# buggyyang/CDC_compression

Hardware: AMD Instinct MI355X
Metric: decoded images/sec at 256x256, 500-step x-param (higher is better)
Workload: dtype f32 (f16x2 split products)

## Files before the change

### cdc_compression_amd/csrc/cdc_internal.h

```cpp
#pragma once
#include <stdio.h>
#include <string.h>
#include <stdlib.h>
#include <hip/hip_runtime.h>
#include <map>
#include <mutex>
#include <utility>
#include <stdint.h>

#include <string>
#include <vector>

#include "conv_args.h"

extern "C" char **environ;

namespace cdc {

typedef void (*conv_kernel_fn)(const ConvArgs);
conv_kernel_fn conv_lookup_a(int MB, int NPW, int lnmode);
conv_kernel_fn conv_lookup_b(int MB, int NPW, int lnmode);
conv_kernel_fn conv_lookup_c(int MB, int NPW, int lnmode);
conv_kernel_fn conv_lookup_split(int MB, int NPW);
conv_kernel_fn conv_lookup_split2(int MB, int NPW, int lnmode, int xu = 1);
conv_kernel_fn conv_lookup_split2h(int MB, int NPW, int lnmode, int xu = 1);
conv_kernel_fn conv_lookup_split2hu(int MB, int NPW);

struct ConvShape {
    int Cin, Cout, KH, KW, stride;
    int C0 = 0;
    int Win = 0;
    int nz = 1, pad_x[4] = {0, 0, 0, 0};
    bool allow_split = false;
    int arith = 0;
    bool per_image_w = false;
    int Ho, Wo;
    int B;
    bool need_all_cout;
    int lnmode;
    int max_ksplit = 1;
};
bool conv_make_plan(const ConvShape &s, ConvPlan *plan);
hipError_t conv_launch(ConvArgs a, const ConvPlan &plan, int B, int nz, hipStream_t st);

struct PfShape {
    int Cin, Cout, C0 = 0, KH, KW, nz = 1, Ho, Wo, B;
    bool need_all_cout = false;
    int stride = 1;
    int uf = 0;
    int cop = 0;
    int tz = 1;
};
struct PfPlan {
    int MB, NPW, WM, WP, ring, tiles_x, tiles_y, groups; size_t lds_bytes; int lin = 0;
    int x16 = 0;
    int pf3_epv = 0, pf3_G = 0, pf3_iters = 0;
};
bool pf_make_plan(const PfShape &s, PfPlan *plan);
hipError_t pf_launch(PfArgs a, const PfPlan &plan, int B, int nz, hipStream_t st);
bool pf3_make_plan(const PfArgs &a, int B, int nz, PfPlan *plan);
hipError_t pf3_launch(PfArgs a, const PfPlan &plan, int B, hipStream_t st);
int device_cus();
struct WsPlan { int W, NPB, stride, waves, tiles, groups; size_t lds_bytes; };
struct WsArgs;
bool ws_make_plan(int Cin, int C0, int Cout, int H, int W, int B, int stride, WsPlan *plan);
hipError_t ws_launch(WsArgs a, const WsPlan &plan, hipStream_t st);
struct Ws1Plan { int NPB, waves, tiles, groups; size_t lds_bytes; };
struct Ws1Args;
bool ws1_make_plan(int Cin, int C0, int Cout, int HW, int B, bool per_image_w, Ws1Plan *plan);
hipError_t ws1_launch(Ws1Args a, const Ws1Plan &plan, hipStream_t st);
bool pw_make_plan(const PfShape &s, PfPlan *plan);
hipError_t pw_launch(PfArgs a, const PfPlan &plan, int B, hipStream_t st);
hipError_t pf_pack_launch(const float *src, long long src_bs, void *dst, long long dst_bs, int C, int H, int W, int B,
                          hipStream_t st);
hipError_t c4_pack_launch(const float *src, long long src_bs, float *dst, int C, long long HW, int B, hipStream_t st);
hipError_t pf_unpack_launch(const void *src, long long src_bs, float *dst, long long dst_bs, int C, int H, int W, int B, hipStream_t st);

inline const char *dev_env(const char *name) {
    static const bool on = [] {
        const char *e = ::getenv("CDC_DEV");
        if (e && atoi(e) != 0) return true;
        static const char *const user_level[] = {"CDC_DEV=", "CDC_ARITH=", "CDC_NO_RANGE_GUARD=", "CDC_GRAPH=", "CDC_DEBUG_PLAN=", "CDC_PROF_OPS=",
                                                 "CDC_BENCH_", "CDC_TEST_OBS=", "CDC_SYNC_EACH_OP=", "CDC_HIP_LIB=", "CDC_NO_COMBINE_FUSE="};
        for (char **v = environ; v && *v; ++v) {
            if (strncmp(*v, "CDC_", 4)) continue;
            bool user = false;
            for (const char *u : user_level) user = user || !strncmp(*v, u, strlen(u));
            if (!user) {
                fprintf(stderr, "cdc_hip: %.*s is set but ignored: development switches need CDC_DEV=1\n", (int)strcspn(*v, "="), *v);
                break;
            }
        }
        return false;
    }();
    return on ? ::getenv(name) : nullptr;
}

inline hipError_t ensure_dynamic_lds(const void *fn, size_t bytes) {
    if (bytes <= 64 * 1024) return hipSuccess;
    static std::mutex mu;
    static std::map<std::pair<int, const void *>, size_t> done;
    int dev = 0;
    (void)hipGetDevice(&dev);
    std::lock_guard<std::mutex> lk(mu);
    size_t &have = done[{dev, fn}];
    if (have >= bytes) return hipSuccess;
    hipError_t e = hipFuncSetAttribute(fn, hipFuncAttributeMaxDynamicSharedMemorySize, (int)bytes);
    if (e == hipSuccess) have = bytes;
    return e;
}

__host__ __device__ inline int ceil_div(int a, int b) { return (a + b - 1) / b; }
__host__ __device__ inline int round_up(int a, int b) { return ceil_div(a, b) * b; }

struct LnArgs {
    const float *in;
    float *out;
    int C, HW;
    const float *g, *b;
    float eps;
    int relu;
    const float *shift;
    int shift_bs;
    const float *resid;
    float *stat_mean, *stat_rstd;
    int nparts;
    long long part_stride;
    int *fault;
    int img_major;
};
hipError_t ln_launch(const LnArgs &a, int B, hipStream_t st);

struct TembLayer {
    const float *w, *bias;
    int cout;
    int out_off;
};
struct TembArgs {
    const float *time;
    const float *w0, *b0;
    const float *w2, *b2;
    int dim;
    const TembLayer *layers;
    int n_layers;
    float *shift;
    int shift_bs;
};
hipError_t temb_launch(const TembArgs &a, int B, hipStream_t st);

struct KvCtxArgs {
    const float *x; long long x_bs;
    const float *mean, *rstd;
    const float *Wt;
    const float *bias;
    const unsigned short *Ws;
    int C, N, nsplit;
    float *S, *Z, *M;
    int f16 = 0;
    float wscale_inv = 1.f;
};
hipError_t kvctx_launch(const KvCtxArgs &a, int B, hipStream_t st);

struct LnConvArgs {
    const float *x; long long x_bs;
    const float *mean, *rstd;
    const unsigned short *Ws;
    const float *bias;
    float *y; long long y_bs;
    int C, N, nsplit;
    void *y_pf = nullptr;
    long long pf_bs = 0, pf_ps = 0;
    int W = 0;
};
hipError_t lnconv_launch(const LnConvArgs &a, int B, hipStream_t st);

hipError_t kstats_launch(const float *k, long long k_bs, int C, int N, float *kmax, int B,
                         hipStream_t st);
hipError_t ctx_partial_launch(const float *k, const float *v, long long kv_bs, int C, int N,
                              const float *kmax, float *S, float *Zp, int nsplit, int B,
                              hipStream_t st, int f16 = 0);
hipError_t ctx_one_launch(const float *k, const float *v, long long kv_bs, int C, int N, float scale, float *ctxw, int Cin_pad, int COP,
                          unsigned short *Ws, int B, hipStream_t st, int f16);
hipError_t ctx_reduce_launch(const float *S, const float *ksum, int C, int nsplit, float scale,
                             float *ctxw, int Cin_pad, int COP, int B, hipStream_t st, unsigned short *Ws = nullptr);

hipError_t ctx_fold_launch(const float *S, const float *ksum, int C, int nsplit, float scale,
                           const float *WoT, const float *WqT, float *T1, float *Mt, int Cin_pad,
                           int COP, const float *ln_g, const float *u, const float *b_out,
                           float *biasB, int B, hipStream_t st, const float *M = nullptr,
                           unsigned short *Ws = nullptr, int ws_f16 = 0, const float *Wq = nullptr);
hipError_t fold_combine_launch(const float *P, const float *bias, float *out, int Cout, int KH,
                               int pad, int H, int W, int B, hipStream_t st);

struct DdimArgs {
    const float *fx, *x, *noise;
    float *x_next;
    const float *tab;
    int steps, i;
    const int *step_ptr;
    int pred_mode, clip;
    float eta;
    long long n;
    long long clip_half_n;
    int *fault;
    const float *tab_v;
    const float *P = nullptr, *P_bias = nullptr;
    int pC = 0, pKH = 0, pPad = 0, pH = 0, pW = 0;
    const unsigned long long *seeds = nullptr;
    long long per_image = 0;
};
hipError_t ddim_launch(const DdimArgs &a, hipStream_t st);
hipError_t randn_fill_launch(const unsigned long long *seeds, int B, long long per_image, unsigned draw, float scale, float *out,
                             hipStream_t st);
hipError_t copy_channels_launch(const float *src, long long src_bs, float *dst, long long dst_bs,
                                long long n, int B, hipStream_t st, int parts = 1, long long part_stride = 0,
                                const int *step_ptr = nullptr, long long step_stride = 0);
hipError_t step_dec_launch(int *step, hipStream_t st);
hipError_t bpp_launch(const float *qh, long long nh, int hw_h, const float *prior, const float *ql, const float *mean,
                      const float *scale, long long nl, float inv_hw, float *bpp, int B, hipStream_t st);
hipError_t clamp_min_launch(float *x, long long bs, long long n, float lo, int B, hipStream_t st);
hipError_t nonfinite_launch(const float *x, long long bs, long long n, int B, int *flag, hipStream_t st);
hipError_t bits_differ_launch(const float *a, const float *b, long long n, long long *counters, hipStream_t st);
hipError_t dequantize_launch(const float *x, const float *loc, float *out, long long n, hipStream_t st);
hipError_t vbr_affine_launch(float *x, long long bs, int C, int HW, const float *rate, const float *p, int leaky, int B, hipStream_t st);
hipError_t frame_in_launch(const void *src, int u8, float *dst, int P, int H, int W, int Hp, int Wp, int zero, hipStream_t st);
hipError_t frame_out_launch(const float *src, void *dst, int u8, int P, int H, int W, int Hp, int Wp, hipStream_t st);
hipError_t unfold_x_launch(const float *src, long long src_bs, float *dst, long long dst_bs, int C, int KW,
                           int pad, int H, int W, int B, hipStream_t st);

}
```

### cdc_compression_amd/csrc/cdc_planner.hip

```cpp
#include "cdc_state.h"

namespace cdcapi {

constexpr int kKsTarget = 1024;

struct Builder {
    cdc_handle *h;
    int B;
    std::vector<void *> *pool;
    int rc = CDC_OK;
    int planB = 0;
    int pb() const { return planB > 0 ? planB : B; }
    std::vector<Op> *cur = nullptr;

    int ws1_h = 0;
    void emit(Op op) {
        op.id = (int)h->op_ms.size();
        h->op_ms.push_back(0); h->op_n.push_back(0); h->op_flops.push_back(op.flops);
        char buf[160];
        const char *kinds[] = {"conv", "ln", "temb", "kstats", "ctxp", "ctxr", "ctxf", "combine", "ddim", "copy", "unfold", "kvctx", "lnconv", "convpf", "pfpack", "convws", "convws1", "vbr"};
        if (op.kind == Op::PFPACK && op.pk.c4 == 2) kinds[Op::PFPACK] = "pfunpack";
        if (op.kind == Op::CONV)
            snprintf(buf, sizeof buf, "conv %dx%d s%d %4d->%-4d out %3dx%-3d MB%d NPW%d WN%d g%d tg%d ipw%d ks%d%s%s%s%s%s", op.conv.KH,
                     op.conv.KW, op.conv.stride, op.conv.Cin, op.conv.Cout, op.conv.Ho, op.conv.Wo, op.plan.MB,
                     op.plan.NPW, op.plan.WN, op.plan.groups, op.plan.tg, op.plan.ipw, op.plan.ksplit, op.plan.split == 2 ? (op.plan.arith ? " SPLIT2H" : " SPLIT2") : (op.plan.split ? " SPLIT" : ""),
                     op.conv.ep_g ? " LN" : "",
                     op.conv.ln_mean ? " pre" : "", cur == &h->pre_ops ? " HOIST" : "", op.conv.resid ? " +res" : "");
        else if (op.kind == Op::CONVPF)
            snprintf(buf, sizeof buf, "conv %dx%d s%d %4d->%-4d out %3dx%-3d MB%d NPW%d WM%d WP%d g%d R%d %s%s%s%s%s%s", op.pf.KH, op.pf.KW,
                     op.pf.stride == 2 ? 2 : 1, op.pf.Cin, op.pf.Cout, op.pf.Ho, op.pf.Wo, op.pfplan.MB, op.pfplan.NPW, op.pfplan.WM, op.pfplan.WP,
                     op.pfplan.groups, op.pfplan.ring, op.pw ? (op.pf.pre_mean ? "PW pre" : "PW") : (op.pfplan.pf3_epv ? (op.pf.ep_g ? "PF3 LN" : "PF3") : (op.pf.ep_g ? "PF LN" : "PF")), op.pf.out ? "" : " nof32", op.pf.out_pf ? " +pf" : "",
                     op.pf.resid ? " +res" : (op.pf.resid_pf ? " +resP" : ""), cur == &h->pre_ops ? " HOIST" : "", op.pf.tz == 4 ? " TZ4" : "");
        else if (op.kind == Op::CONVWS)
            snprintf(buf, sizeof buf, "conv 3x3 s%d %4d->%-4d out %3dx%-3d NPB%d waves%d tiles%d g%d WS%s", op.wsplan.stride, op.ws.Cin, op.ws.Cout, op.ws.H, op.wsplan.W,
                     op.wsplan.NPB, op.wsplan.waves, op.wsplan.tiles, op.wsplan.groups, op.ws.pre_add ? " pre_add" : "");
        else if (op.kind == Op::CONVWS1)
            snprintf(buf, sizeof buf, "conv 1x1 s1 %4d->%-4d out %3dx%-3d NPB%d waves%d tiles%d g%d WS1%s%s%s", op.ws1.Cin, op.ws1.Cout, ws1_h, op.ws1.HW / std::max(ws1_h, 1),
                     op.ws1plan.NPB, op.ws1plan.waves, op.ws1plan.tiles, op.ws1plan.groups, op.ws1.pre_mean ? " pre" : "", op.ws1.w_bs ? " perimg" : "",
                     op.ws1.resid ? (op.ws1.resid_is_pre ? " pre_add" : " +res") : "");
        else if (op.kind == Op::LN)
            snprintf(buf, sizeof buf, "ln C=%d HW=%d%s", op.ln.C, op.ln.HW, op.ln.out ? "" : " stats");
        else if (op.kind == Op::KVCTX)
            snprintf(buf, sizeof buf, "kvctx C=%d N=%d nsplit=%d", op.kvc.C, op.kvc.N, op.kvc.nsplit);
        else if (op.kind == Op::LNCONV)
            snprintf(buf, sizeof buf, "lnconv C=%d N=%d nsplit=%d", op.lnc.C, op.lnc.N, op.lnc.nsplit);
        else if (op.kind == Op::VBR)
            snprintf(buf, sizeof buf, "vbr C=%d HW=%d%s", op.vb.C, op.vb.HW, op.vb.leaky ? " leaky" : "");
        else if (op.kind == Op::KSTATS || op.kind == Op::CTXP || op.kind == Op::CTXR || op.kind == Op::CTXF)
            snprintf(buf, sizeof buf, "%s C=%d N=%d nsplit=%d", op.at_one ? "ctx1" : kinds[op.kind], op.at.C, op.at.N, op.at_one ? 1 : op.at.nsplit);
        else
            snprintf(buf, sizeof buf, "%s", kinds[op.kind]);
        if (cur == &h->pre_ops && !strstr(buf, " HOIST") && strlen(buf) + 7 < sizeof buf) strcat(buf, " HOIST");
        h->op_label.push_back(buf);
        (cur ? cur : &h->ops)->push_back(op);
    }

    int *fault_flag() {
        if (!h->d_fault && !rc) {
            void *p = nullptr;
            hipError_t e = hipMalloc(&p, sizeof(int));
            if (e == hipSuccess) e = hipMemset(p, 0, sizeof(int));
            if (e != hipSuccess) { rc = fail(h, CDC_ERR_NOMEM, "range-guard flag: %s", hipGetErrorString(e)); return nullptr; }
            h->d_fault = (int *)p;
            h->weight_allocs.push_back(p);
        }
        return h->d_fault;
    }

    float *dalloc(size_t nfloats) {
        if (rc) return nullptr;
        void *p = nullptr;
        const size_t bytes = std::max<size_t>(nfloats, 1) * sizeof(float);
        hipError_t e = hipMalloc(&p, bytes);
        if (e != hipSuccess) {
            rc = fail(h, CDC_ERR_NOMEM, "hipMalloc(%zu bytes) failed: %s", bytes, hipGetErrorString(e));
            return nullptr;
        }
        pool->push_back(p);
        h->act_bytes += bytes;
        return (float *)p;
    }
    struct PfTwin { void *p = nullptr; int C = 0, H = 0, W = 0; bool valid = false;
                    bool only = false;
                    long long ps() const { return (long long)(H + 2) * (W + 2); }
                    long long bs() const { return (long long)(C / 8) * 2 * ps(); } };
    std::map<const float *, PfTwin> pfmap;
    enum Site { SITE_NONE, SITE_ALWAYS, SITE_RB_CHAIN, SITE_DOWN, SITE_JOIN, SITE_ALWAYS_PLANES };
    int pf_mode() const { const char *e = dev_env("CDC_PF"); return h->arith != 1 ? 0 : (e ? atoi(e) : 3); }
    bool pf_site(Site s, int H, int W) const {
        const int m = pf_mode();
        if (m == 1) return s != SITE_NONE;
        if (m != 3) return false;
        const long long join_max = 16384;
        return s == SITE_RB_CHAIN || s == SITE_DOWN || s == SITE_ALWAYS_PLANES || (s == SITE_JOIN && (long long)H * W <= join_max);
    }
    bool pf_on() const { return pf_mode() != 0; }
    static long long pf_maxpix() { const char *e = dev_env("CDC_PF_MAXPIX"); const long long v = e ? atoll(e) : 0; return v > 0 ? v : (1LL << 40); }
    PfTwin *twin(const float *p) { auto it = pfmap.find(p); return it == pfmap.end() ? nullptr : &it->second; }
    bool still_planes_only(const float *p) { PfTwin *t = twin(p); return t && t->only; }
    void add_twin(const float *p, int C, int H, int W) {
        if (rc || !p || !pf_on() || (C % 16) || W < 32 || H < 2 || (long long)H * W > pf_maxpix()) return;
        PfTwin t; t.C = C; t.H = H; t.W = W;
        const size_t bytes = (size_t)B * t.bs() * 16;
        void *q = nullptr;
        hipError_t e = hipMalloc(&q, bytes);
        if (e == hipSuccess) e = hipMemset(q, 0, bytes);
        if (e != hipSuccess) { rc = fail(h, CDC_ERR_NOMEM, "PF tensor (%zu bytes): %s", bytes, hipGetErrorString(e)); return; }
        pool->push_back(q);
        h->act_bytes += bytes;
        t.p = q;
        pfmap[p] = t;
    }
    void pack(const float *p, long long bs) {
        PfTwin *t = twin(p);
        if (rc || !t) return;
        Op op; op.kind = Op::PFPACK; op.prof = PC_SMALL;
        op.pk = {p, bs, t->p, t->bs(), t->C, t->H, t->W, 0};
        op.bytes = 8.0 * B * t->C * t->H * t->W;
        emit(op);
        t->valid = true;
    }
    bool ensure_f32(const float *q, long long bs) {
        PfTwin *t = q ? twin(q) : nullptr;
        if (!t || !t->only) return true;
        if (rc || !t->valid || bs != (long long)t->C * t->H * t->W) return false;
        Op op; op.kind = Op::PFPACK; op.prof = PC_SMALL;
        op.pk = {q, bs, t->p, t->bs(), t->C, t->H, t->W, 2};
        op.bytes = 8.0 * B * t->C * t->H * t->W;
        emit(op);
        t->only = false;
        ++n_unpacked;
        if (debug_plan()) fprintf(stderr, "[plan] planes-only tensor %dx%dx%d unpacked for an fp32 reader\n", t->C, t->H, t->W);
        return true;
    }
    int n_unpacked = 0;

    std::map<const float *, float *> c4map;
    const float *pre_add_c4(const float *p, int C, int H, int W, long long bs) {
        if (rc || (C % 4) || bs != (long long)C * H * W || dev_env("CDC_NO_PRE_C4")) return nullptr;
        auto it = c4map.find(p);
        if (it != c4map.end()) return it->second;
        float *q = dalloc((size_t)B * C * H * W);
        if (rc) return nullptr;
        std::vector<Op> *saved = cur;
        cur = &h->pre_ops;
        Op op; op.kind = Op::PFPACK; op.prof = PC_SMALL;
        op.pk = {p, bs, q, 0, C, H, W, 1};
        op.bytes = 8.0 * B * C * H * W;
        emit(op);
        cur = saved;
        c4map[p] = q;
        return q;
    }
    Act new_act(int C, int H, int W, bool want_twin = true, Site site = SITE_ALWAYS) {
        Act a; a.C = C; a.H = H; a.W = W;
        a.p = dalloc((size_t)B * C * H * W);
        if (want_twin && pf_site(site, H, W)) add_twin(a.p, C, H, W);
        return a;
    }

    struct ConvOpts {
        const float *ln_g = nullptr, *ln_b = nullptr;
        int relu = 0;
        float relu_slope = 0.f;
        const float *shift = nullptr;
        const float *resid = nullptr; long long resid_bs = 0, resid_cs = 0;
        const float *resid1 = nullptr; long long resid1_bs = 0; int resid_c0 = 0;
        const float *pre_add = nullptr;
        float *stat_mean = nullptr, *stat_rstd = nullptr;
        const float *pre_mean = nullptr, *pre_rstd = nullptr, *pre_g = nullptr, *pre_b = nullptr;
        int pre_mode = 1;
        int shift_bs = -1;
        long long w_bs = 0;
        long long wsp_bs = 0;
        bool no_bias = false;
        const float *res3_w = nullptr, *res3_x = nullptr; long long res3_bs = 0;
        int max_ksplit = 1;
        bool emit_pf = false;
        bool pf_only = false;
        bool no_f32 = false;
        int uf_c = 0, uf_pad = 0;
        bool linear_epilogue() const { return !ln_g && !relu && !shift && !stat_mean && !pre_add && !res3_w; }
    };
    int last_ksplit = 1;
    bool last_pf_only = false;
    const float *next_res3_w = nullptr, *next_res3_x = nullptr; long long next_res3_bs = 0;
    static bool debug_plan() { return getenv("CDC_DEBUG_PLAN") != nullptr; }

    PfShape pf_shape(const ConvW &w, int C0, int Ho, int Wo, bool need_all) const {
        PfShape ps;
        ps.Cin = w.Cin; ps.Cout = w.Cout; ps.C0 = C0; ps.KH = w.KH; ps.KW = w.KW; ps.nz = w.nz; ps.Ho = Ho; ps.Wo = Wo; ps.B = pb();
        ps.need_all_cout = need_all; ps.cop = w.COP;
        return ps;
    }
    bool pf_form(const ConvW &w, int C0, int H, int W, bool need_all, PfShape *ps) const {
        if (!w.wsh || w.stride != 1 || w.transposed || (w.Cin % 16) || !((w.KH == 3 && w.KW == 3) || (w.KH == 1 && w.KW == 1))) return false;
        if (w.py() != w.KH / 2 || w.px() != w.KW / 2) return false;
        *ps = pf_shape(w, C0, H, W, need_all);
        return true;
    }
    bool pf_s2_form(const ConvW &w, int C0, int H, int W, bool need_all, PfShape *ps) const {
        if (!w.wsh || w.stride != 2 || w.transposed || w.KH != 3 || w.KW != 3 || C0 || (H & 1) || (W & 1) || (w.Cin % 16)) return false;
        if (w.py() != 1 || w.px() != 1) return false;
        *ps = pf_shape(w, 0, H / 2, W / 2, need_all);
        ps->stride = 2;
        return true;
    }
    bool pf_tz_form(const ConvW &w, int C0, int H, int W, bool need_all, PfShape *ps) const {
        if (!w.wsh || !w.transposed || w.tk != 4 || w.KH != 2 || w.KW != 2 || C0 || (w.Cin % 16)) return false;
        *ps = pf_shape(w, 0, H, W, need_all);
        ps->tz = 4;
        return true;
    }
    bool pf_17_form(const ConvW &w, int C0, int H, int W, bool need_all, PfShape *ps) const {
        if (!w.wsh || w.KH != 1 || w.KW != 7 || w.stride != 1 || w.transposed || C0 || (w.Cin % 16)) return false;
        if (w.py() != 0 || w.px() != 3) return false;
        *ps = pf_shape(w, 0, H, W, need_all);
        return true;
    }
    bool pf_uf_form(const ConvW &w, int H, int W, bool need_all, PfShape *ps) const {
        if (!w.wsh || w.KH != 7 || w.KW != 1 || w.stride != 1 || w.transposed || w.nz != 1 || w.py() != 3 || w.px() != 0) return false;
        *ps = pf_shape(w, 0, H, W, need_all);
        ps->uf = 3;
        return true;
    }
    bool pw_form(const ConvW &w, int C0, int H, int W, PfShape *ps) const {
        if (!w.wsh || w.KH != 1 || w.KW != 1 || w.stride != 1 || w.transposed || w.nz != 1 || w.py() != 0 || w.px() != 0) return false;
        *ps = pf_shape(w, C0, H, W, false);
        return true;
    }
    static bool pf_plans(const PfShape &ps) { PfPlan plan; return pf_make_plan(ps, &plan); }

    bool pf_would_plan(const ConvW &w, int H, int W) { PfShape ps; return pf_on() && pf_form(w, 0, H, W, true, &ps) && pf_plans(ps); }
    bool pf_s2_would_plan(const ConvW &w, int H, int W) { PfShape ps; return pf_on() && pf_s2_form(w, 0, H, W, false, &ps) && pf_plans(ps); }
    bool pf_tz_would_plan(const ConvW &w, int H, int W) { PfShape ps; return pf_on() && pf_tz_form(w, 0, H, W, false, &ps) && pf_plans(ps); }
    bool pf_17_would_plan(const ConvW &w, int H, int W) { PfShape ps; return pf_on() && pf_17_form(w, 0, H, W, false, &ps) && pf_plans(ps); }

    bool join_reads_planes(const ResBlockW &rb, const float *p0, int C0, const float *p1, int H, int W) {
        PfTwin *t0 = twin(p0), *t1 = twin(p1);
        if (!t0 || !t1 || !t1->valid || t0->H != H || t0->W != W || t1->H != H || t1->W != W) return false;
        if (t0->C != C0 || t0->C + t1->C != rb.c1.Cin) return false;
        return join_would_read_planes(rb, C0, H, W);
    }
    bool join_would_read_planes(const ResBlockW &rb, int C0, int H, int W) {
        if (!pf_on() || !rb.has_res || rb.hoist_cx) return false;
        if (rb.cres.Cin != rb.c1.Cin || (C0 % 16) || C0 <= 0 || C0 >= rb.c1.Cin || !pf_site(SITE_JOIN, H, W)) return false;
        PfShape p1, pr;
        return pf_form(rb.c1, C0, H, W, rb.c1.KH == 3, &p1) && pf_plans(p1) && pf_form(rb.cres, C0, H, W, rb.cres.KH == 3, &pr) && pf_plans(pr);
    }

    template <class A> static void out_geometry(A &a, const ConvW &w, int Ho, int Wo) {
        if (w.transposed) {
            for (int z = 0; z < 4; ++z) {
                const int py = z >> 1, px = z & 1;
                a.pad_y[z] = w.tk == 5 ? 1 : 1 - py; a.pad_x[z] = w.tk == 5 ? 1 : 1 - px;
                a.out_zoff[z] = py * 2 * Wo + px;
            }
            a.out_cs = (long long)4 * Ho * Wo; a.out_ys = 4 * Wo; a.out_xs = 2;
        } else {
            a.pad_y[0] = w.py(); a.pad_x[0] = w.px();
            a.out_cs = (long long)Ho * Wo; a.out_ys = Wo; a.out_xs = 1;
        }
        a.Ho = Ho; a.Wo = Wo;
    }
    PfTwin *out_twin(const float *out, long long bs, int C, int H, int W) {
        PfTwin *t = twin(out);
        return t && t->C == C && t->H == H && t->W == W && bs == (long long)C * H * W ? t : nullptr;
    }
    template <class A> bool bind_out_pf(A &a, const ConvW &w, const float *out, long long out_bs, int Ho, int Wo) {
        const int Wt = w.transposed ? 2 * Wo : Wo;
        PfTwin *to = out_twin(out, out_bs, w.Cout, w.transposed ? 2 * Ho : Ho, Wt);
        if (!to) return false;
        a.out_pf = to->p; a.pf_bs = to->bs(); a.pf_ps = to->ps();
        if (w.transposed) {
            a.pf_ys = 2 * (Wt + 2); a.pf_xs = 2;
            for (int z = 0; z < 4; ++z) a.pf_zoff[z] = ((z >> 1) + 1) * (Wt + 2) + (z & 1) + 1;
        } else {
            a.pf_ys = Wt + 2; a.pf_xs = 1; a.pf_zoff[0] = (Wt + 2) + 1;
        }
        to->valid = true;
        return true;
    }
    int shift_stride(const ConvOpts &o) const { return o.shift_bs >= 0 ? o.shift_bs : h->shift_bs; }
    template <class A> void epilogue(A &a, const ConvW &w, const ConvOpts &o) {
        a.bias = o.no_bias ? nullptr : w.bias;
        a.pre_add = o.pre_add;
        a.ep_g = o.ln_g; a.ep_b = o.ln_b; a.eps = 1e-5f; a.relu = o.relu; a.relu_slope = o.relu_slope;
        a.shift = o.shift; a.shift_bs = shift_stride(o);
        a.resid = o.resid; a.resid_bs = o.resid_bs; a.resid_cs = o.resid_cs;
        a.stat_mean = o.stat_mean; a.stat_rstd = o.stat_rstd;
        a.res3_w = o.res3_w; a.res3_x = o.res3_x; a.res3_bs = o.res3_bs;
        a.fault = fault_flag();
    }
    bool finish(Op &op, double flops, double bytes, bool pf_only) {
        op.flops = flops; op.bytes = bytes;
        last_ksplit = 1;
        last_pf_only = pf_only;
        emit(op);
        return true;
    }

    bool try_pf(const ConvW &w, const float *s0, int C0, const float *s1, int H, int W, float *out, long long out_bs,
                const ConvOpts &o, bool need_all, int prof) {
        if (!pf_on() || o.pre_mean || o.w_bs || o.wsp_bs || o.max_ksplit > 1) return false;
        PfShape ps;
        const int c0 = s1 ? C0 : 0;
        if (!(pf_form(w, c0, H, W, need_all, &ps) || (pf_s2_form(w, c0, H, W, need_all, &ps) && !o.pre_add && !o.res3_w) ||
              pf_tz_form(w, c0, H, W, need_all, &ps) || (pf_17_form(w, c0, H, W, need_all, &ps) && !o.ln_g && !o.emit_pf)))
            return false;
        if (s1 && dev_env("CDC_TEST_JOIN_MISS")) return false;
        PfTwin *t0 = twin(s0), *t1 = s1 ? twin(s1) : nullptr;
        if (!t0 || !t0->valid || (s1 && (!t1 || !t1->valid))) return false;
        if (t0->H != H || t0->W != W || (t1 && (t1->H != H || t1->W != W))) return false;
        if (s1 ? (t0->C != C0 || t0->C + t1->C != w.Cin) : t0->C != w.Cin) return false;
        PfPlan plan;
        if (!pf_make_plan(ps, &plan)) return false;
        const int Ho = ps.Ho, Wo = ps.Wo;
        Op op;
        op.kind = Op::CONVPF; op.prof = prof; op.pfplan = plan; op.nz = w.nz;
        PfArgs &a = op.pf;
        memset(&a, 0, sizeof a);
        a.src0 = t0->p; a.src0_bs = t0->bs();
        if (t1) { a.src1 = t1->p; a.src1_bs = t1->bs(); }
        a.C0 = s1 ? C0 : w.Cin; a.Cin = w.Cin; a.H = H; a.W = W;
        a.w = w.wsh; a.w_zs = w.wsp_zs / 8;
        a.KH = w.KH; a.KW = w.KW; a.nz = w.nz; a.stride = w.stride; a.tz = ps.tz;
        a.nchunk = w.Cin / 16; a.COP = w.COP; a.Cout = w.Cout;
        a.acc_scale = w.wscale_inv;
        out_geometry(a, w, Ho, Wo);
        a.out = out; a.out_bs = out_bs;
        if (o.emit_pf && bind_out_pf(a, w, out, out_bs, Ho, Wo) && o.no_f32) a.out = nullptr;
        epilogue(a, w, o);
        if (o.resid1) {
            if (!o.resid || o.resid_c0 <= 0 || o.resid_c0 >= w.Cout || (o.resid_c0 % 64) || (o.resid_c0 % (plan.MB * 32))) return false;
            a.resid1 = o.resid1; a.resid1_bs = o.resid1_bs; a.resid_c0 = o.resid_c0;
        }
        if (PfTwin *tr = o.resid ? twin(o.resid) : nullptr)
            if (tr->only) {
                if (!tr->valid || tr->C != w.Cout || tr->H != Ho || tr->W != Wo || w.transposed || w.stride != 1 ||
                    o.resid_bs != (long long)w.Cout * Ho * Wo || o.resid_cs != (long long)Ho * Wo) {
                    if (!ensure_f32(o.resid, o.resid_bs)) {
                        if (!rc) rc = fail(h, CDC_ERR_UNSUPPORTED, "planes-only residual of a shape the plane-operand kernels do not read");
                        return true;
                    }
                } else {
                    a.resid = nullptr;
                    a.resid_pf = tr->p; a.rpf_bs = tr->bs(); a.rpf_ps = tr->ps(); a.rpf_ys = Wo + 2; a.rpf_zoff = (Wo + 2) + 1;
                }
            }
        if (planB == 0) pf3_make_plan(a, B, w.nz, &op.pfplan);
        if (debug_plan())
            fprintf(stderr, "[plan] conv %dx%d %d->%d out %dx%d on conv_pf%s_kernel (epv %d, %d workgroups x %d tiles per group)\n", w.KH, w.KW, w.Cin, w.Cout,
                    Ho, Wo, op.pfplan.pf3_epv ? "3" : "", op.pfplan.pf3_epv, op.pfplan.pf3_G, op.pfplan.pf3_iters);
        const double px = (double)B * Ho * Wo * w.nz;
        return finish(op, 2.0 * px * w.Cout * w.Cin * w.KH * w.KW, 4.0 * ((double)B * w.Cin * H * W + px * w.Cout), a.out == nullptr);
    }

    bool try_pf_uf(const ConvW &w, const float *s0, long long bs0, int H, int W, float *out, long long out_bs, const ConvOpts &o,
                   bool need_all, int prof) {
        PfShape ps;
        if (!pf_on() || o.uf_c != 3 || o.uf_pad != 3 || !pf_uf_form(w, H, W, need_all, &ps)) return false;
        if (o.pre_mean || o.w_bs || o.wsp_bs || o.max_ksplit > 1 || o.resid || o.res3_w || o.stat_mean) return false;
        PfPlan plan;
        if (!pf_make_plan(ps, &plan)) return false;
        Op op;
        op.kind = Op::CONVPF; op.prof = prof; op.pfplan = plan; op.nz = 1;
        PfArgs &a = op.pf;
        memset(&a, 0, sizeof a);
        a.x0 = s0; a.x0_bs = bs0;
        a.C0 = a.Cin = 32; a.H = H; a.W = W;
        a.w = w.wsh; a.w_zs = w.wsp_zs / 8;
        a.KH = 7; a.KW = 1; a.nz = 1;
        a.nchunk = 2; a.COP = w.COP; a.Cout = w.Cout;
        a.acc_scale = w.wscale_inv;
        out_geometry(a, w, H, W);
        a.out = out; a.out_bs = out_bs;
        if (o.emit_pf && bind_out_pf(a, w, out, out_bs, H, W) && o.no_f32) a.out = nullptr;
        const float *c4 = o.pre_add && cur != &h->pre_ops ? pre_add_c4(o.pre_add, w.Cout, H, W, out_bs) : nullptr;
        epilogue(a, w, o);
        if (c4) { a.pre_add = c4; a.pre_c4 = 1; }
        const double px = (double)B * H * W;
        return finish(op, 2.0 * px * w.Cout * w.Cin * 7, 4.0 * ((double)B * 3 * H * W + px * w.Cout), a.out == nullptr);
    }

    bool try_pw(const ConvW &w, const float *s0, int C0, long long bs0, const float *s1, long long bs1, int H, int W,
                float *out, long long out_bs, const ConvOpts &o, bool need_all, int prof) {
        PfShape ps;
        if (h->arith != 1 || dev_env("CDC_NO_PW") || !pw_form(w, s1 ? C0 : 0, H, W, &ps)) return false;
        if (need_all || o.ln_g || o.stat_mean || o.res3_w || o.pf_only) return false;
        if (o.pre_mean && o.pre_mode != 2) return false;
        if (o.w_bs && !o.wsp_bs) return false;
        PfPlan plan;
        if (!pw_make_plan(ps, &plan)) return false;
        if (plan.lin && (o.shift || o.wsp_bs || (long long)w.Cout * H * W != out_bs)) return false;
        if (debug_plan())
            fprintf(stderr, "[plan] conv1x1 PW Cin=%4d Cout=%4d out=%3dx%-3d %s%s| MB=%d NPW=%d WM=%d WP=%d groups=%d R=%d wgs=%d lds=%zu\n", w.Cin, w.Cout,
                    H, W, o.pre_mean ? "pre2 " : "", o.wsp_bs ? "per-image " : "", plan.MB, plan.NPW, plan.WM, plan.WP, plan.groups, plan.ring,
                    plan.tiles_x * plan.tiles_y * B * plan.groups, plan.lds_bytes);
        Op op;
        op.kind = Op::CONVPF; op.prof = prof; op.pfplan = plan; op.nz = 1; op.pw = true;
        PfArgs &a = op.pf;
        memset(&a, 0, sizeof a);
        a.x0 = s0; a.x0_bs = bs0; a.x1 = s1; a.x1_bs = bs1;
        a.C0 = s1 ? C0 : w.Cin; a.Cin = w.Cin; a.H = H; a.W = W;
        a.pre_mean = o.pre_mean; a.pre_rstd = o.pre_mean ? o.pre_rstd : nullptr;
        a.w = w.wsh; a.w_bs = o.wsp_bs / 8;
        a.KH = 1; a.KW = 1; a.nz = 1;
        a.nchunk = w.Cin / 16; a.COP = w.COP; a.Cout = w.Cout;
        a.acc_scale = w.wscale_inv;
        out_geometry(a, w, H, W);
        a.out = out; a.out_bs = out_bs;
        if (o.emit_pf && !plan.lin && (w.Cout % 32) == 0 && bind_out_pf(a, w, out, out_bs, H, W) && o.no_f32) a.out = nullptr;
        epilogue(a, w, o);
        const double px = (double)B * H * W;
        return finish(op, 2.0 * px * w.Cout * w.Cin, 4.0 * ((double)B * w.Cin * H * W + px * w.Cout), a.out == nullptr);
    }

    bool ws_would_plan(const ConvW &w, int C0, bool two_src, int H, int W, WsPlan *plan) {
        if (h->arith != 1 || !w.wsh || planB > 0 || w.KH != 3 || w.KW != 3 || (w.stride != 1 && w.stride != 2) || w.transposed || w.nz != 1) return false;
        if (w.py() != 1 || w.px() != 1) return false;
        if (w.COP != w.Cout || w.Cin_pad != w.Cin) return false;
        if (w.stride == 2 && ((H & 1) || (W & 1) || two_src)) return false;
        return ws_make_plan(w.Cin, two_src ? C0 : w.Cin, w.Cout, H / w.stride, W / w.stride, pb(), w.stride, plan);
    }
    bool try_ws(const ConvW &w, const float *s0, int C0, long long bs0, const float *s1, long long bs1, int H, int W, float *raw,
                long long raw_bs, int prof, const float *pre_add = nullptr) {
        Op op;
        op.kind = Op::CONVWS; op.prof = prof;
        if (rc || !ws_would_plan(w, C0, s1 != nullptr, H, W, &op.wsplan)) return false;
        if (!ensure_f32(s0, bs0) || (s1 && !ensure_f32(s1, bs1))) return false;
        const int Ho = H / w.stride, Wo = W / w.stride;
        if (raw_bs != (long long)w.Cout * Ho * Wo) return false;
        WsArgs &a = op.ws;
        memset(&a, 0, sizeof a);
        a.x0 = s0; a.x0_bs = bs0; a.x1 = s1; a.x1_bs = bs1;
        a.C0 = s1 ? C0 : w.Cin; a.Cin = w.Cin; a.H = Ho; a.B = B;
        a.w = w.wsh; a.nchunk = w.Cin / 16; a.COP = w.COP; a.Cout = w.Cout; a.acc_scale = w.wscale_inv;
        a.bias = pre_add ? nullptr : w.bias;
        a.pre_add = pre_add;
        a.out = raw; a.out_bs = raw_bs;
        a.fault = fault_flag();
        if (debug_plan())
            fprintf(stderr, "[plan] conv 3x3 s%d %d->%d out %dx%d on conv_ws_kernel: %d tiles of %d pixels x %d groups, %d waves, %zu bytes of LDS\n", w.stride, w.Cin, w.Cout, Ho, Wo,
                    op.wsplan.tiles, op.wsplan.NPB * 32, op.wsplan.groups, op.wsplan.waves, op.wsplan.lds_bytes);
        const double px = (double)B * Ho * Wo;
        return finish(op, 2.0 * px * w.Cout * w.Cin * 9, 4.0 * ((double)B * H * W * w.Cin + px * w.Cout), false);
    }

    bool try_ws1(const ConvW &w, const float *s0, int C0, long long bs0, const float *s1, long long bs1, int H, int W, float *out, long long out_bs,
                 const ConvOpts &o, bool need_all, int prof) {
        PfShape ps;
        if (rc || h->arith != 1 || planB > 0 || !pw_form(w, 0, H, W, &ps)) return false;
        if (need_all || o.ln_g || o.stat_mean || o.res3_w || o.pf_only || (o.pre_add && o.resid) || o.relu || o.resid1 || o.uf_c) return false;
        if (o.pre_mean && o.pre_mode != 2) return false;
        if (o.w_bs && !o.wsp_bs) return false;
        if (w.COP != w.Cout || w.Cin_pad != w.Cin || out_bs != (long long)w.Cout * H * W) return false;
        if (o.resid && (o.resid_cs != (long long)H * W)) return false;
        const long long blocks = (long long)pb() * (H * W / 32);
        const long long max_blocks = dev_env("CDC_WS1_MAX_BLOCKS") ? atoll(dev_env("CDC_WS1_MAX_BLOCKS")) : 128;
        const int max_groups_wide = dev_env("CDC_WS1_MAX_GROUPS") ? atoi(dev_env("CDC_WS1_MAX_GROUPS")) : 0;
        const bool wide_ok = blocks <= max_blocks || (max_groups_wide > 0 && blocks <= 256 && w.Cout / 32 <= max_groups_wide);
        if (!wide_ok && !(o.wsp_bs && W < 32)) return false;
        Op op;
        op.kind = Op::CONVWS1; op.prof = prof;
        if (!ws1_make_plan(w.Cin, s1 ? C0 : w.Cin, w.Cout, H * W, pb(), o.wsp_bs != 0, &op.ws1plan)) return false;
        if (!ensure_f32(s0, bs0) || (s1 && !ensure_f32(s1, bs1)) || (o.resid && !ensure_f32(o.resid, o.resid_bs))) return false;
        Ws1Args &a = op.ws1;
        memset(&a, 0, sizeof a);
        a.x0 = s0; a.x0_bs = bs0; a.x1 = s1; a.x1_bs = bs1;
        a.C0 = s1 ? C0 : w.Cin; a.Cin = w.Cin; a.HW = H * W; a.B = B;
        a.pre_mean = o.pre_mean; a.pre_rstd = o.pre_mean ? o.pre_rstd : nullptr;
        a.w = w.wsh; a.w_bs = o.wsp_bs / 8;
        a.nchunk = w.Cin / 16; a.COP = w.COP; a.Cout = w.Cout; a.acc_scale = w.wscale_inv;
        a.bias = o.no_bias ? nullptr : w.bias;
        a.shift = o.shift; a.shift_bs = shift_stride(o);
        a.resid = o.resid; a.resid_bs = o.resid_bs;
        if (o.pre_add) { a.resid = o.pre_add; a.resid_bs = out_bs; a.resid_is_pre = 1; }
        a.out = out; a.out_bs = out_bs;
        a.fault = fault_flag();
        if (debug_plan())
            fprintf(stderr, "[plan] conv 1x1 %d->%d out %dx%d on conv_ws1_kernel: %d tiles of %d pixels x %d groups, %d waves%s%s\n", w.Cin, w.Cout, H, W,
                    op.ws1plan.tiles, op.ws1plan.NPB * 32, op.ws1plan.groups, op.ws1plan.waves, o.pre_mean ? ", folded PreNorm" : "", o.wsp_bs ? ", per-image weights" : "");
        ws1_h = H;
        const double px = (double)B * H * W;
        return finish(op, 2.0 * px * w.Cout * w.Cin, 4.0 * px * (w.Cin + w.Cout), false);
    }

    bool conv(const ConvW &w, const float *s0, int C0, long long bs0, const float *s1,
              long long bs1, int H, int W, float *out, long long out_bs, const ConvOpts &o,
              bool need_all, int prof) {
        if (rc) return true;
        if (s1 && (C0 % 4)) {
            const long long n0 = (long long)C0 * H * W, n1 = (long long)(w.Cin - C0) * H * W;
            float *cat = dalloc((size_t)B * (n0 + n1));
            copy(s0, bs0, cat, n0 + n1, n0);
            copy(s1, bs1, cat + n0, n0 + n1, n1);
            s0 = cat; bs0 = n0 + n1; s1 = nullptr; bs1 = 0;
        }
        ConvShape s;
        s.Cin = w.Cin; s.Cout = w.Cout; s.KH = w.KH; s.KW = w.KW; s.stride = w.stride;
        s.C0 = s1 ? C0 : 0;
        s.Win = W; s.nz = w.nz;
        s.allow_split = w.wsp != nullptr;
        s.arith = (h->arith == 1 && w.wsh) ? 1 : 0;
        s.per_image_w = o.wsp_bs != 0;
        for (int z = 0; z < 4; ++z) s.pad_x[z] = w.transposed ? (w.tk == 5 ? 1 : 1 - (z & 1)) : w.px();
        if (w.transposed) { s.Ho = H; s.Wo = W; }
        else {
            s.Ho = (H + 2 * w.py() - w.KH) / w.stride + 1;
            s.Wo = (W + 2 * w.px() - w.KW) / w.stride + 1;
        }
        s.B = pb(); s.need_all_cout = need_all; s.lnmode = o.pre_mean ? o.pre_mode : 0;
        if (!o.uf_c && try_pf(w, s0, C0, s1, H, W, out, out_bs, o, need_all, prof)) return true;
        if (o.uf_c && !s1 && try_pf_uf(w, s0, bs0, H, W, out, out_bs, o, need_all, prof)) return true;
        if (o.pf_only) return false;
        if (o.resid1 && !rc) { rc = fail(h, CDC_ERR_UNSUPPORTED, "a two-source residual reached a kernel without it"); return true; }
        {
            const std::pair<const float *, long long> rd[3] = {{s0, bs0}, {s1, bs1}, {o.resid, o.resid_bs}};
            for (const auto &q : rd)
                if (!ensure_f32(q.first, q.second) && !rc) {
                    rc = fail(h, CDC_ERR_UNSUPPORTED, "a planes-only tensor reached a kernel that reads fp32 and cannot be unpacked");
                    return true;
                }
        }
        if (w.stride == 2 && !need_all && o.linear_epilogue() && !o.resid && !o.pre_mean && !o.w_bs && !o.uf_c && !(o.emit_pf && twin(out)) &&
            try_ws(w, s0, C0, bs0, s1, bs1, H, W, out, out_bs, prof))
            return true;
        if (!o.uf_c && try_ws1(w, s0, C0, bs0, s1, bs1, H, W, out, out_bs, o, need_all, prof)) return true;
        if (!o.uf_c && try_pw(w, s0, C0, bs0, s1, bs1, H, W, out, out_bs, o, need_all, prof)) return true;
        const bool linear_ep = !need_all && o.linear_epilogue() && w.nz == 1 && !w.transposed;
        s.max_ksplit = o.max_ksplit > 1 ? o.max_ksplit : (linear_ep ? 4 : 1);
        if (need_all && (w.Cout % 32)) return false;
        ConvPlan plan;
        if (!conv_make_plan(s, &plan)) {
            if (need_all) return false;
            rc = fail(h, CDC_ERR_UNSUPPORTED, "no launch plan for conv Cin=%d Cout=%d k=%dx%d out=%dx%d",
                      w.Cin, w.Cout, w.KH, w.KW, s.Ho, s.Wo);
            return true;
        }
        if (o.uf_c && !(plan.split == 2 && plan.arith == 1 && plan.xu == 1 && plan.lnmode == 0 &&
                        conv_lookup_split2hu(plan.MB, plan.NPW))) return false;
        last_ksplit = 1;
        last_pf_only = false;
        if (o.max_ksplit > 1 && plan.split == 2 && !need_all) {
            const long long wgs = (long long)(plan.ipw > 1 ? ceil_div(pb(), plan.ipw) : plan.tiles_x * plan.tiles_y * pb()) *
                                  plan.groups * w.nz;
            int ks = (int)std::min<long long>(ceil_div(kKsTarget, wgs), std::min(o.max_ksplit, plan.nchunk / 4));
            if (ks > 1) { plan.ksplit = ks; last_ksplit = ks; }
        }
        float *ks_scratch = nullptr;
        const long long dense_bs = (long long)w.Cout * s.Ho * s.Wo;
        if (o.max_ksplit <= 1 && plan.split == 2 && linear_ep) {
            const long long wgs = (long long)(plan.ipw > 1 ? ceil_div(pb(), plan.ipw) : plan.tiles_x * plan.tiles_y * pb()) *
                                  plan.groups;
            const int ks = (int)std::min<long long>(ceil_div(kKsTarget, wgs), std::min(4, plan.nchunk / 4));
            if (ks > 1 && (planB > 0 || (size_t)B * dense_bs * 4 * ks <= (64u << 20))) {
                plan.ksplit = ks;
                ks_scratch = dalloc((size_t)ks * B * dense_bs);
            }
        }
        if (debug_plan())
            fprintf(stderr, "[plan] %-10s Cin=%4d Cout=%4d k=%dx%d s=%d in=%3dx%-3d out=%3dx%-3d %s%s%s| MB=%2d NPW=%d "
                    "WN=%d groups=%2d KC=%2d nchunk=%3d tiles=%dx%d wgs=%6d lds=%6zu\n", kProfNames[prof], w.Cin,
                    w.Cout, w.KH, w.KW, w.stride, H, W, s.Ho, s.Wo, need_all ? "LN " : "   ",
                    s.lnmode ? (s.lnmode == 2 ? "pre2 " : "pre1 ") : "     ", cur == &h->pre_ops ? "HOIST " : "", plan.MB, plan.NPW, plan.WN,
                    plan.groups, plan.KC, plan.nchunk, plan.tiles_x, plan.tiles_y,
                    plan.tiles_x * plan.tiles_y * B * plan.groups * w.nz, plan.lds_bytes);
        Op op;
        op.kind = Op::CONV; op.prof = prof; op.plan = plan; op.nz = w.nz;
        ConvArgs &a = op.conv;
        memset(&a, 0, sizeof a);
        a.src0 = s0; a.src1 = s1; a.src0_bs = bs0; a.src1_bs = bs1;
        a.C0 = s1 ? C0 : w.Cin; a.Cin = w.Cin; a.H = H; a.W = W;
        a.ln_mean = o.pre_mean; a.ln_rstd = o.pre_rstd; a.ln_g = o.pre_g; a.ln_b = o.pre_b;
        a.wp = w.wp; a.w_bs = o.w_bs; a.w_zs = w.w_zs;
        a.wsp = w.wsp; a.wsp_zs = w.wsp_zs; a.wsp_bs = o.wsp_bs;
        a.acc_scale = 1.f;
        if (plan.split == 2 && plan.arith == 1) { a.wsp = w.wsh; a.acc_scale = w.wscale_inv; }
        a.KH = w.KH; a.KW = w.KW; a.stride = w.stride;
        a.Cin_pad = w.Cin_pad; a.COP = w.COP; a.Cout = w.Cout;
        a.out = out; a.out_bs = out_bs; a.out_ks = (long long)B * out_bs;
        out_geometry(a, w, s.Ho, s.Wo);
        epilogue(a, w, o);
        if (o.uf_c) {
            a.uf_c = o.uf_c; a.uf_pad = o.uf_pad;
            a.uf_magic = o.uf_c > 1 ? (unsigned)(((1ull << 32) + o.uf_c - 1) / o.uf_c) : 0u;
        }
        if (o.emit_pf && !ks_scratch && plan.ksplit <= 1 && (w.Cout % 32) == 0 && bind_out_pf(a, w, out, out_bs, s.Ho, s.Wo)) {
            a.pf_only = o.no_f32 ? 1 : 0;
            last_pf_only = o.no_f32;
        }
        const double px = (double)B * s.Ho * s.Wo * w.nz;
        op.flops = 2.0 * px * w.Cout * w.Cin * w.KH * w.KW;
        op.bytes = 4.0 * ((double)B * w.Cin * H * W + px * w.Cout);
        if (ks_scratch) {
            a.out = ks_scratch; a.out_bs = dense_bs; a.out_ks = (long long)B * dense_bs;
        }
        emit(op);
        if (ks_scratch) {
            Op c; c.kind = Op::COPY; c.prof = prof;
            c.cp = {ks_scratch, dense_bs, out, out_bs, dense_bs};
            c.cp_parts = plan.ksplit; c.cp_part_stride = (long long)B * dense_bs;
            c.bytes = 4.0 * B * dense_bs * (plan.ksplit + 1);
            emit(c);
            if (o.emit_pf && !w.transposed && out_twin(out, out_bs, w.Cout, s.Ho, s.Wo)) pack(out, out_bs);
        }
        return true;
    }

    void ln(const float *in, float *out, int C, int HW, const float *g, const float *b, int relu,
            const float *shift, const float *resid, float *sm, float *sr, int nparts = 1) {
        if (rc) return;
        Op op;
        op.kind = Op::LN; op.prof = PC_LN;
        LnArgs &a = op.ln;
        a.nparts = nparts; a.part_stride = (long long)B * C * HW;
        a.in = in; a.out = out; a.C = C; a.HW = HW; a.g = g; a.b = b; a.eps = 1e-5f; a.relu = relu;
        a.shift = shift; a.shift_bs = h->shift_bs; a.resid = resid; a.stat_mean = sm; a.stat_rstd = sr;
        a.fault = fault_flag();
        op.bytes = 4.0 * B * C * HW * (out ? 2 : 1);
        emit(op);
    }

    void copy(const float *src, long long src_bs, float *dst, long long dst_bs, long long n) {
        Op c; c.kind = Op::COPY; c.prof = PC_SMALL;
        c.cp = {src, src_bs, dst, dst_bs, n};
        c.bytes = 8.0 * B * n;
        emit(c);
    }

    bool prefer_fused(const ConvW &w, int H, int W) {
        if (w.Cout % 32 || w.Cout > 384) return false;
        if (w.wsp && w.Cout > 256 && (W & 3) == 0 && !dev_env("CDC_NO_SPLIT")) return false;
        ConvShape s;
        s.Cin = w.Cin; s.Cout = w.Cout; s.KH = w.KH; s.KW = w.KW; s.stride = w.stride;
        s.Ho = H; s.Wo = W; s.B = pb(); s.lnmode = 0;
        s.Win = W; s.pad_x[0] = w.pad;
        ConvPlan pf, pu;
        s.need_all_cout = true;
        if (!conv_make_plan(s, &pf)) return false;
        s.need_all_cout = false;
        if (!conv_make_plan(s, &pu)) return true;
        const double wf = (double)pf.tiles_x * pf.tiles_y * B * pf.WN;
        const double wu = (double)pu.tiles_x * pu.tiles_y * B * pu.groups * pu.WN;
        static const double thr = 512;
        if (wf >= thr) return true;
        return wu < 1.5 * wf;
    }

    bool block(const ConvW &w, const float *s0, int C0, long long bs0, const float *s1, long long bs1,
               int H, int W, Act out, const float *g, const float *b, const float *shift,
               const float *pre_add, const float *resid, long long resid_bs, float *sm, float *sr,
// ... 769 lines not shown
```

### cdc_compression_amd/csrc/conv_inst_p.hip

```cpp
#include <algorithm>
#include <map>
#include <string>
#include <vector>
#include <stdlib.h>

#include "cdc_internal.h"
#include "conv_pf_kernel.h"

namespace cdc {

template <int KH, int KW>
static pf_kernel_fn pf_lookup_k(int MB, int NPW, int WM, int WP) {
    if (MB == 2 && NPW == 2 && WM == 1 && WP == 4) return conv_pf_kernel<2, 2, 1, 4, KH, KW>;
    if (MB == 2 && NPW == 2 && WM == 2 && WP == 2) return conv_pf_kernel<2, 2, 2, 2, KH, KW>;
    if (MB == 2 && NPW == 2 && WM == 2 && WP == 4) return conv_pf_kernel<2, 2, 2, 4, KH, KW>;
    if (MB == 3 && NPW == 2 && WM == 2 && WP == 4) return conv_pf_kernel<3, 2, 2, 4, KH, KW>;
    if (MB == 3 && NPW == 1 && WM == 2 && WP == 4 && KH == 3) return conv_pf_kernel<3, 1, 2, 4, KH, KW>;
    if (MB == 2 && NPW == 2 && WM == 4 && WP == 2) return conv_pf_kernel<2, 2, 4, 2, KH, KW>;
    return nullptr;
}
static pf_kernel_fn pf_lookup_s2(int MB, int NPW, int WM, int WP) {
    if (MB == 2 && NPW == 1 && WM == 1 && WP == 4) return conv_pf_kernel<2, 1, 1, 4, 3, 3, 2>;
    if (MB == 2 && NPW == 2 && WM == 2 && WP == 2) return conv_pf_kernel<2, 2, 2, 2, 3, 3, 2>;
    if (MB == 3 && NPW == 1 && WM == 2 && WP == 4) return conv_pf_kernel<3, 1, 2, 4, 3, 3, 2>;
    return nullptr;
}
static pf_kernel_fn pf_lookup_tz(int MB, int NPW, int WM, int WP) {
    if (MB == 1 && NPW == 2 && WM == 2 && WP == 2) return conv_pf_kernel<1, 2, 2, 2, 2, 2, 1, 4>;
    if (MB == 2 && NPW == 1 && WM == 1 && WP == 4) return conv_pf_kernel<2, 1, 1, 4, 2, 2, 1, 4>;
    if (MB == 1 && NPW == 2 && WM == 4 && WP == 2) return conv_pf_kernel<1, 2, 4, 2, 2, 2, 1, 4>;
    return nullptr;
}
static pf_kernel_fn pf_lookup(int MB, int NPW, int WM, int WP, int KH, int KW, int stride = 1, int tz = 1) {
    if (tz == 4) return (KH == 2 && KW == 2 && stride != 2) ? pf_lookup_tz(MB, NPW, WM, WP) : nullptr;
    if (stride == 2) return (KH == 3 && KW == 3) ? pf_lookup_s2(MB, NPW, WM, WP) : nullptr;
    if (KH == 3 && KW == 3) return pf_lookup_k<3, 3>(MB, NPW, WM, WP);
    if (KH == 1 && KW == 1) return pf_lookup_k<1, 1>(MB, NPW, WM, WP);
    if (KH == 2 && KW == 2) return pf_lookup_k<2, 2>(MB, NPW, WM, WP);
    if (KH == 1 && KW == 7 && MB == 1 && NPW == 2 && WM == 1 && WP == 4) return conv_pf_kernel<1, 2, 1, 4, 1, 7>;
    if (KH == 7 && KW == 1 && MB == 2 && NPW == 2 && WM == 1 && WP == 4) return conv_pf_kernel<2, 2, 1, 4, 7, 1, 1, 1, 3>;
    return nullptr;
}

struct PfCand { int MB, NPW, WM, WP; };
static const PfCand kCandsS2[] = {
    {2, 2, 2, 2},
    {3, 1, 2, 4},
    {2, 1, 1, 4},
};
static const PfCand kCandsTZ[] = {
    {1, 2, 4, 2},
    {2, 1, 1, 4},
    {1, 2, 2, 2},
};
static const PfCand kCands[] = {
    {2, 2, 4, 2},
    {3, 2, 2, 4},
    {3, 1, 2, 4},
    {2, 2, 2, 2},
    {2, 2, 2, 4},
    {2, 2, 1, 4},
};

bool pf_make_plan(const PfShape &s, PfPlan *p) {
    if (s.uf) {
        if (s.uf != 3 || s.KH != 7 || s.KW != 1 || s.Cin != 21 || s.Cout != 64 || s.cop != 64 || s.C0 || s.nz != 1 || s.stride != 1 || s.tz != 1 ||
            s.Wo < 32 || dev_env("CDC_NO_PF_UF"))
            return false;
        const int ring = pf_ring(2, 2, 1, 4, 7, 1);
        const double wgs = (double)((s.Wo + 31) / 32) * ((s.Ho + 7) / 8) * s.B;
        const double min_wgs = dev_env("CDC_PF_UF_MIN_WGS") ? atof(dev_env("CDC_PF_UF_MIN_WGS")) : 512.0;
        if (ring < 3 || wgs < min_wgs) return false;
        p->MB = 2; p->NPW = 2; p->WM = 1; p->WP = 4; p->ring = ring;
        p->tiles_x = (s.Wo + 31) / 32; p->tiles_y = (s.Ho + 7) / 8; p->groups = 1;
        p->lds_bytes = (size_t)2 * pf_patch_units(2, 4, 7, 1) * 16 + (size_t)ring * pf_rows(2, 2) * 64 * 16 + (size_t)pf_uf_stage_floats(2, 4) * 4;
        return true;
    }
    if (s.KH == 1 && s.KW == 7) {
        if (s.Cout > 32 || s.cop != 32 || s.Cin % 16 || s.C0 || s.nz != 1 || s.stride != 1 || s.tz != 1 || s.need_all_cout || s.Wo < 32 ||
            dev_env("CDC_NO_PF_17"))
            return false;
        const int ring = pf_ring(1, 2, 1, 4, 1, 7);
        const double wgs = (double)((s.Wo + 31) / 32) * ((s.Ho + 7) / 8) * s.B;
        const double min_wgs = dev_env("CDC_PF_17_MIN_WGS") ? atof(dev_env("CDC_PF_17_MIN_WGS")) : 768.0;
        if (!ring || (s.Cin / 16) * 7 < ring - 1 || wgs < min_wgs) return false;
        p->MB = 1; p->NPW = 2; p->WM = 1; p->WP = 4; p->ring = ring;
        p->tiles_x = (s.Wo + 31) / 32; p->tiles_y = (s.Ho + 7) / 8; p->groups = 1;
        p->lds_bytes = (size_t)2 * pf_patch_units(2, 4, 1, 7) * 16 + (size_t)ring * pf_rows(1, 2) * 32 * 16;
        return true;
    }
    if (s.Cout % 32 || s.Cin % 16 || (s.C0 % 16)) return false;
    if (s.Wo < 32) return false;
    const char *force = dev_env("CDC_PF_PLAN");
    int f[4] = {0, 0, 0, 0};
    if (force) sscanf(force, "%d,%d,%d,%d", &f[0], &f[1], &f[2], &f[3]);
    double best = -1;
    if (s.stride == 2) {
        if (s.KH != 3 || s.KW != 3 || s.nz != 1 || s.C0 || dev_env("CDC_NO_PF_S2")) return false;
        for (const PfCand &c : kCandsS2) {
            if (f[0] && (c.MB != f[0] || c.NPW != f[1] || c.WM != f[2] || c.WP != f[3])) continue;
            const int COPT = c.WM * c.MB * 32, TH = c.WP * c.NPW;
            if (s.Cout % COPT || (s.need_all_cout && COPT != s.Cout)) continue;
            const int ring = pf_ring(c.MB, c.NPW, c.WM, c.WP, 3, 3, 2);
            const int tps = pf_tps(c.MB, c.NPW, c.WM, c.WP, 3, 3, 2);
            const int S = (s.Cin / 16) * 9 / tps;
            if (!ring || S < ring - 1) continue;
            const double wgs = (double)((s.Wo + 31) / 32) * ((s.Ho + TH - 1) / TH) * s.B * (s.Cout / COPT);
            const double min_wgs = dev_env("CDC_PF_S2_MIN_WGS") ? atof(dev_env("CDC_PF_S2_MIN_WGS")) : 128.0;
            if (wgs < min_wgs) continue;
            const double score = (double)COPT;
            if (score <= best) continue;
            best = score;
            const size_t patch = (size_t)pf_patch_bufs(3, 3, 2) * pf_patch_units(c.NPW, c.WP, 3, 3, 2) * 16, wst = (size_t)tps * pf_rows(c.MB, c.NPW) * COPT * 16;
            p->MB = c.MB; p->NPW = c.NPW; p->WM = c.WM; p->WP = c.WP;
            p->ring = ring;
            p->tiles_x = (s.Wo + 31) / 32; p->tiles_y = (s.Ho + TH - 1) / TH;
            p->groups = s.Cout / COPT;
            p->lds_bytes = std::max(patch + ring * wst, sizeof(float) * (size_t)(4 * COPT + 2 * c.WM * c.WP * c.NPW * 32));
        }
        return best >= 0;
    }
    if (s.tz == 4) {
        if (s.KH != 2 || s.KW != 2 || s.C0 || dev_env("CDC_NO_PF_TZ")) return false;
        for (const PfCand &c : kCandsTZ) {
            if (f[0] && (c.MB != f[0] || c.NPW != f[1] || c.WM != f[2] || c.WP != f[3])) continue;
            const int COPT = c.WM * c.MB * 32, TH = c.WP * c.NPW;
            if (COPT != s.Cout) continue;
            const int ring = pf_ring(c.MB, c.NPW, c.WM, c.WP, 2, 2, 1, 4);
            const int tps = pf_tps(c.MB, c.NPW, c.WM, c.WP, 2, 2, 1, 4);
            const int S = (s.Cin / 16) * 16 / tps;
            if (!ring || S < ring - 1) continue;
            const double wgs = (double)((s.Wo + 31) / 32) * ((s.Ho + TH - 1) / TH) * s.B;
            const double min_wgs = dev_env("CDC_PF_TZ_MIN_WGS") ? atof(dev_env("CDC_PF_TZ_MIN_WGS")) : 128.0;
            if (wgs < min_wgs) continue;
            best = COPT;
            const size_t patch = (size_t)2 * pf_patch_units(c.NPW, c.WP, 2, 2, 1, 4) * 16, wst = (size_t)tps * pf_rows(c.MB, 4 * c.NPW) * COPT * 16;
            p->MB = c.MB; p->NPW = c.NPW; p->WM = c.WM; p->WP = c.WP;
            p->ring = ring;
            p->tiles_x = (s.Wo + 31) / 32; p->tiles_y = (s.Ho + TH - 1) / TH;
            p->groups = 1;
            p->lds_bytes = std::max(patch + ring * wst, sizeof(float) * (size_t)(4 * COPT + 2 * c.WM * c.WP * 4 * c.NPW * 32));
            break;
        }
        return best >= 0;
    }
    for (const PfCand &c : kCands) {
        if (f[0] && (c.MB != f[0] || c.NPW != f[1] || c.WM != f[2] || c.WP != f[3])) continue;
        const int COPT = c.WM * c.MB * 32, NW = c.WM * c.WP;
        if (s.Cout % COPT) continue;
        if (s.need_all_cout && COPT != s.Cout) continue;
        if (!pf_lookup(c.MB, c.NPW, c.WM, c.WP, s.KH, s.KW)) continue;
        const int TH = c.WP * c.NPW, PH = TH + s.KH - 1, PW = 32 + s.KW - 1;
        const int xsw = (4 * PH * PW + 63) / 64;
        if (xsw > 2 * kPfXS) continue;
        const int taps = s.KH * s.KW, npb = taps == 1 ? 3 : 2;
        const size_t patch = (size_t)npb * xsw * 64 * 16, wst = (size_t)pf_rows(c.MB, c.NPW) * COPT * 16;
        const int ring = pf_ring(c.MB, c.NPW, c.WM, c.WP, s.KH, s.KW);
        if (!ring) continue;
        const int S = (s.Cin / 16) * taps;
        if (S < ring - 1) continue;
        const double wgs = (double)((s.Wo + 31) / 32) * ((s.Ho + TH - 1) / TH) * s.B * (s.Cout / COPT) * s.nz;
        const double min_waves = dev_env("CDC_PF_MIN_WAVES") ? atof(dev_env("CDC_PF_MIN_WAVES")) : 256.0;
        if (wgs * NW < min_waves) continue;
        if (c.MB == 3 && c.NPW == 1 && wgs < 128.0) continue;
        const double fill = std::min(1.0, wgs * NW / 2048.0);
        const double reads = (3.0 * c.MB + 2.0 * c.NPW) / (3.0 * c.MB * c.NPW);
        const double score = fill * (1.0 - 0.35 * reads) * (s.Cout / COPT > 1 ? 0.9 : 1.0);
        if (score > best) {
            best = score;
            p->MB = c.MB; p->NPW = c.NPW; p->WM = c.WM; p->WP = c.WP;
            p->ring = ring;
            p->tiles_x = (s.Wo + 31) / 32; p->tiles_y = (s.Ho + TH - 1) / TH;
            p->groups = s.Cout / COPT;
            p->lds_bytes = std::max(patch + ring * wst, sizeof(float) * (size_t)(4 * COPT + 2 * c.WM * c.WP * c.NPW * 32));
        }
    }
    return best >= 0;
}

hipError_t pf_launch(PfArgs a, const PfPlan &p, int B, int nz, hipStream_t st) {
    if (p.pf3_epv) return pf3_launch(a, p, B, st);
    pf_kernel_fn fn = pf_lookup(p.MB, p.NPW, p.WM, p.WP, a.KH, a.KW, a.stride == 2 ? 2 : 1, a.tz == 4 ? 4 : 1);
    if (!fn) return hipErrorInvalidValue;
    if (a.tz == 4) nz = 1;
    a.lognbw = 5;
    a.dbg = 0;
    a.tiles_x = p.tiles_x; a.tiles_y = p.tiles_y; a.B = B; a.ring = p.ring;
    if (hipError_t e = ensure_dynamic_lds((const void *)fn, p.lds_bytes); e != hipSuccess) return e;
    dim3 grid((unsigned)(p.tiles_x * p.tiles_y * B), (unsigned)p.groups, (unsigned)nz);
    a.xcd_remap = (grid.x % 8 == 0 && grid.x >= 64) ? 1 : 0;
#ifdef CDC_TIMELINE
    static unsigned long long *tl_dev = nullptr;
    static std::map<std::string, int> seen;
    const size_t tl_wgs = (size_t)grid.x * grid.y * grid.z;
    char key[96];
    snprintf(key, sizeof key, "%dx%d s%d tz%d %d->%d out %dx%d", a.KH, a.KW, a.stride == 2 ? 2 : 1, a.tz == 4 ? 4 : 1, a.Cin, a.Cout, a.Ho, a.Wo);
    a.tl = nullptr;
    if (tl_wgs <= (1u << 18) && seen[key]++ < 3) {
        if (!tl_dev) hipMalloc(&tl_dev, sizeof(unsigned long long) * 16 * (1u << 18));
        hipMemsetAsync(tl_dev, 0, sizeof(unsigned long long) * 16 * tl_wgs, st);
        a.tl = tl_dev;
    }
#endif
    hipLaunchKernelGGL(fn, grid, dim3(64 * p.WM * p.WP), p.lds_bytes, st, a);
#ifdef CDC_TIMELINE
    if (a.tl) {
        hipStreamSynchronize(st);
        std::vector<unsigned long long> h(16 * tl_wgs);
        hipMemcpy(h.data(), tl_dev, h.size() * 8, hipMemcpyDeviceToHost);
        unsigned long long t0 = ~0ull, t1 = 0;
        double cat[7] = {0}, life = 0;
        std::map<unsigned long long, int> per_cu;
        std::vector<unsigned long long> starts;
        for (size_t w = 0; w < tl_wgs; ++w) {
            const unsigned long long *r = &h[w * 16];
            for (int c = 0; c < 7; ++c) cat[c] += (double)r[c];
            t0 = std::min(t0, r[7]); t1 = std::max(t1, r[8]);
            life += (double)(r[8] - r[7]);
            per_cu[(r[10] & 0xf) << 32 | (r[9] & 0xffff00)]++;
            starts.push_back(r[7]);
        }
        std::sort(starts.begin(), starts.end());
        int cu_min = 1 << 30, cu_max = 0;
        for (auto &kv : per_cu) { cu_min = std::min(cu_min, kv.second); cu_max = std::max(cu_max, kv.second); }
        static const char *names[7] = {"setup", "prologue issue", "prologue wait", "main loop", "epilogue parameters", "epilogue arithmetic", "epilogue stores"};
        fprintf(stderr, "[pf timeline] conv %s: %zu workgroups x %d threads, lds %zu; kernel span %llu cycles, mean workgroup life %.0f; %zu CUs used, %d .. %d workgroups per CU;"
                        " start of the median / last workgroup at %llu / %llu; per workgroup (wave 0):", key, tl_wgs, 64 * p.WM * p.WP, p.lds_bytes, t1 - t0, life / tl_wgs,
                per_cu.size(), cu_min, cu_max, starts[starts.size() / 2] - t0, starts.back() - t0);
        for (int c = 0; c < 7; ++c) fprintf(stderr, "  %s %.0f", names[c], cat[c] / tl_wgs);
        fprintf(stderr, "\n");
    }
#endif
    return hipGetLastError();
}

__global__ void __launch_bounds__(256) pf_pack_kernel(const float *src, long long src_bs, uint4 *dst, long long dst_bs,
                                                      int C, int H, int W) {
    const int b = blockIdx.y;
    const long long n = (long long)(C / 8) * H * W;
    const long long i = (long long)blockIdx.x * 256 + threadIdx.x;
    if (i >= n) return;
    const int x = (int)(i % W);
    const long long t = i / W;
    const int y = (int)(t % H), g = (int)(t / H);
    const float *sp = src + (size_t)b * src_bs + ((size_t)g * 8 * H + y) * W + x;
    f16x8 hv, lv;
#pragma unroll
    for (int q = 0; q < 8; ++q) {
        _Float16 h, l;
        split2h(sp[(size_t)q * H * W], h, l);
        hv[q] = h; lv[q] = l;
    }
    const long long ps = (long long)(H + 2) * (W + 2);
    uint4 *dp = dst + (size_t)b * dst_bs + (long long)g * 2 * ps + (long long)(y + 1) * (W + 2) + x + 1;
    dp[0] = __builtin_bit_cast(uint4, hv);
    dp[ps] = __builtin_bit_cast(uint4, lv);
}

hipError_t pf_pack_launch(const float *src, long long src_bs, void *dst, long long dst_bs, int C, int H, int W, int B,
                          hipStream_t st) {
    const long long n = (long long)(C / 8) * H * W;
    dim3 grid((unsigned)((n + 255) / 256), (unsigned)B);
    hipLaunchKernelGGL(pf_pack_kernel, grid, dim3(256), 0, st, src, src_bs, reinterpret_cast<uint4 *>(dst), dst_bs, C, H, W);
    return hipGetLastError();
}

__global__ void __launch_bounds__(256) c4_pack_kernel(const float *src, long long src_bs, float4 *dst, int C, long long HW) {
    const int b = blockIdx.y;
    const long long n = (long long)(C / 4) * HW;
    const long long i = (long long)blockIdx.x * 256 + threadIdx.x;
    if (i >= n) return;
    const long long pix = i % HW, g = i / HW;
    const float *sp = src + (size_t)b * src_bs + (size_t)g * 4 * HW + pix;
    dst[(size_t)b * n + i] = make_float4(sp[0], sp[HW], sp[2 * HW], sp[3 * HW]);
}

hipError_t c4_pack_launch(const float *src, long long src_bs, float *dst, int C, long long HW, int B, hipStream_t st) {
    const long long n = (long long)(C / 4) * HW;
    dim3 grid((unsigned)((n + 255) / 256), (unsigned)B);
    hipLaunchKernelGGL(c4_pack_kernel, grid, dim3(256), 0, st, src, src_bs, reinterpret_cast<float4 *>(dst), C, HW);
    return hipGetLastError();
}

__global__ void __launch_bounds__(256) pf_unpack_kernel(const uint4 *src, long long src_bs, float *dst, long long dst_bs, int C, int H, int W) {
    const int b = blockIdx.y;
    const long long n = (long long)(C / 8) * H * W;
    const long long i = (long long)blockIdx.x * 256 + threadIdx.x;
    if (i >= n) return;
    const int x = (int)(i % W);
    const long long t = i / W;
    const int y = (int)(t % H), g = (int)(t / H);
    const long long ps = (long long)(H + 2) * (W + 2);
    const uint4 *sp = src + (size_t)b * src_bs + (long long)g * 2 * ps + (long long)(y + 1) * (W + 2) + x + 1;
    const f16x8 hv = __builtin_bit_cast(f16x8, sp[0]), lv = __builtin_bit_cast(f16x8, sp[ps]);
    float *dp = dst + (size_t)b * dst_bs + ((size_t)g * 8 * H + y) * W + x;
#pragma unroll
    for (int q = 0; q < 8; ++q) dp[(size_t)q * H * W] = (float)hv[q] + (float)lv[q] * (1.0f / 2048.0f);
}

hipError_t pf_unpack_launch(const void *src, long long src_bs, float *dst, long long dst_bs, int C, int H, int W, int B, hipStream_t st) {
    const long long n = (long long)(C / 8) * H * W;
    dim3 grid((unsigned)((n + 255) / 256), (unsigned)B);
    hipLaunchKernelGGL(pf_unpack_kernel, grid, dim3(256), 0, st, reinterpret_cast<const uint4 *>(src), src_bs, dst, dst_bs, C, H, W);
    return hipGetLastError();
}

}
```

### cdc_compression_amd/csrc/conv_pf_kernel.h

```cpp
#pragma once
#include <type_traits>

#include "conv_split_kernel.h"

namespace cdc {


#ifndef CDC_DMA_WAIT_MARGIN
#define CDC_DMA_WAIT_MARGIN 1
#endif
#ifdef CDC_DMA_WAIT_ALL
constexpr int kVmWaitMask = 0;
#else
constexpr int kVmWaitMask = ~0;
#endif
template <int N> __device__ __forceinline__ void vm_wait() { asm volatile("s_waitcnt vmcnt(%0)" ::"n"(N & kVmWaitMask) : "memory"); }

__device__ __forceinline__ void dma16(unsigned voff, const void *sbase, unsigned lds_byte) {
    asm volatile("s_mov_b32 m0, %2\n\ts_nop 0\n\tglobal_load_lds_dwordx4 %0, %1" ::"v"(voff), "s"(sbase), "s"(lds_byte)
                 : "memory");
}

template <int N, class F> __device__ __forceinline__ void static_for(F &&f) {
    if constexpr (N > 0) {
        static_for<N - 1>(f);
        f(std::integral_constant<int, N - 1>{});
    }
}

__host__ __device__ constexpr bool pf_acc2(int MB, int NPW) { return MB * NPW <= 4; }
__host__ __device__ constexpr int pf_rows(int MB, int NPW) { return pf_acc2(MB, NPW) ? 4 : 6; }
__host__ __device__ constexpr int pf_patch_units(int NPW, int WP, int KH, int KW, int STR = 1, int TZ = 1) {
    return TZ == 4 ? ((4 * (WP * NPW + 2) * 34 + 63) / 64) * 64 : ((4 * ((WP * NPW - 1) * STR + KH) * (31 * STR + KW) + 63) / 64) * 64;
}
__host__ __device__ constexpr int pf_uf_stage_floats(int NPW, int WP) { return ((3 * (WP * NPW + 6) * 38 + 63) / 64) * 64; }
#ifndef CDC_PF_S2_NPB
#define CDC_PF_S2_NPB 2
#endif
__host__ __device__ constexpr int pf_patch_bufs(int KH, int KW, int STR = 1) { return STR == 2 ? CDC_PF_S2_NPB : (KH * KW == 1 ? 3 : 2); }
__host__ __device__ constexpr int pf_ring_tps(int MB, int NPW, int WM, int WP, int KH, int KW, int STR, int tps, int TZ = 1) {
    const size_t budget = ((WM * WP == 8 || STR == 2) ? 156 * 1024 : 80 * 1024) - ((KH == 7 && KW == 1) ? pf_uf_stage_floats(NPW, WP) * 4 : 0);
    const size_t patch = (size_t)pf_patch_bufs(KH, KW, STR) * pf_patch_units(NPW, WP, KH, KW, STR, TZ) * 16;
    const size_t wst = (size_t)tps * pf_rows(MB, TZ * NPW) * WM * MB * 32 * 16;
#ifndef CDC_PF_RING_MAX
#define CDC_PF_RING_MAX 5
#endif
    for (int r = CDC_PF_RING_MAX; r >= 3; --r)
        if (patch + r * wst <= budget) return r;
    return 0;
}
#ifndef CDC_PF_S2_TPS
#define CDC_PF_S2_TPS 3
#endif
#ifndef CDC_PF_TZ_MINB
#define CDC_PF_TZ_MINB 2
#endif
#ifndef CDC_PF_TZ_TPS
#define CDC_PF_TZ_TPS 2
#endif
__host__ __device__ constexpr int pf_tps(int MB, int NPW, int WM, int WP, int KH, int KW, int STR = 1, int TZ = 1) {
    if (TZ == 4) return (CDC_PF_TZ_TPS > 1 && pf_ring_tps(MB, NPW, WM, WP, KH, KW, STR, CDC_PF_TZ_TPS, TZ) >= 3) ? CDC_PF_TZ_TPS : 1;
    return (STR == 2 && CDC_PF_S2_TPS > 1 && pf_ring_tps(MB, NPW, WM, WP, KH, KW, STR, CDC_PF_S2_TPS) >= 3) ? CDC_PF_S2_TPS : 1;
}
__host__ __device__ constexpr int pf_ring(int MB, int NPW, int WM, int WP, int KH, int KW, int STR = 1, int TZ = 1) {
    return pf_ring_tps(MB, NPW, WM, WP, KH, KW, STR, pf_tps(MB, NPW, WM, WP, KH, KW, STR, TZ), TZ);
}
#ifndef CDC_PF_ABLATE
#define CDC_PF_ABLATE 0
#endif

template <int MB, int NPW, int WM, int WP, int KH, int KW, int STR = 1, int TZ = 1, int UF = 0>
__global__ void __launch_bounds__(64 * WM * WP, (KH == 1 && KW == 7) ? 3 : STR == 2 ? 1 : ((WM * WP == 8 || MB * NPW * TZ <= 4 || (TZ == 4 && MB * NPW <= 2 && CDC_PF_TZ_MINB == 2)) ? 2 : 1)) conv_pf_kernel(const PfArgs P) {
    constexpr int NW = WM * WP, NT = 64 * NW, COPT = WM * MB * 32;
    static_assert(COPT % 64 == 0 || COPT == 32, "a weight DMA instruction (64 units) must stay inside one (plane, k-half) row");
    static_assert(TZ == 1 || (TZ == 4 && KH == 2 && KW == 2 && STR == 1), "fused phases: the 2x2 phase form of the 4x4 transposed convolution");
    constexpr int NB = TZ * NPW;
    constexpr bool ACC2 = pf_acc2(MB, NB);
    constexpr int NPL = ACC2 ? 2 : 3, ROWS = 2 * NPL;
    constexpr int WI = (ROWS * COPT + 63) / 64;
    constexpr int NWV = NW - 2;
    constexpr int NWW = (WI + NWV - 1) / NWV;
    constexpr int TAPZ = KH * KW, TAPS = TAPZ * TZ;
    constexpr int NBW = 32, NBH = 1;
    constexpr int TH = WP * NPW * NBH;
    constexpr int PH = TZ == 4 ? TH + 2 : (TH - 1) * STR + KH, PW = TZ == 4 ? NBW + 2 : (NBW - 1) * STR + KW, PLANE = PH * PW;
    constexpr int NE = (PW + 1) / 2;
    constexpr int NX = 4 * PLANE;
    constexpr int XSW = (NX + 63) / 64;
    constexpr int KX = (XSW + 1) / 2;
    constexpr int PST = XSW * 64;
    constexpr int NPB = pf_patch_bufs(KH, KW, STR), LA = NPB - 1;
    constexpr int TPS = pf_tps(MB, NPW, WM, WP, KH, KW, STR, TZ);
    static_assert(TAPZ % TPS == 0, "a weight stage is a whole number of taps of one chunk (and of one phase)");
    constexpr int SPC = TAPS / TPS;
    constexpr int TAPW = ROWS * COPT;
    constexpr int WST = TPS * TAPW;
    static_assert(UF != 0 || KX <= (STR == 2 ? 20 : kPfXS), "patch too large for two patch waves");
    static_assert(UF == 0 || (UF == 3 && KH == 7 && KW == 1 && STR == 1 && TZ == 1 && NPB == 2), "UF: the 7x1 form of the first layer");
    static_assert(STR == 1 || (STR == 2 && KH == 3 && KW == 3), "stride 2 is the 3x3 Downsample form");
    extern __shared__ __attribute__((aligned(16))) uint4 smem_u[];
#ifdef CDC_TIMELINE
    unsigned long long tl_acc[7] = {0, 0, 0, 0, 0, 0, 0}, tl_last = __builtin_readcyclecounter();
    const unsigned long long tl_start = tl_last;
#define PFTL(c) do { const unsigned long long n_ = __builtin_readcyclecounter(); tl_acc[c] += n_ - tl_last; tl_last = n_; } while (0)
#define PFTL_END() do { if (P.tl && threadIdx.x == 0) { unsigned long long *r_ = P.tl + 16 * ((size_t)blockIdx.x + (size_t)gridDim.x * (blockIdx.y + (size_t)gridDim.y * blockIdx.z)); \
        for (int c_ = 0; c_ < 7; ++c_) r_[c_] = tl_acc[c_]; r_[7] = tl_start; r_[8] = __builtin_readcyclecounter(); \
        unsigned hw_; asm volatile("s_getreg_b32 %0, hwreg(HW_REG_HW_ID)" : "=s"(hw_)); r_[9] = hw_; \
        unsigned xcc_; asm volatile("s_getreg_b32 %0, hwreg(HW_REG_XCC_ID)" : "=s"(xcc_)); r_[10] = xcc_; } } while (0)
#else
#define PFTL(c) do { } while (0)
#define PFTL_END() do { } while (0)
#endif
    const int tid = threadIdx.x, lane = tid & 63;
    const int wave = __builtin_amdgcn_readfirstlane(tid >> 6);
    const int wm = wave / WP, wp = wave % WP;
    const bool patch_wave = wave >= NWV;
    const int pwi = wave - NWV;
    const int z = blockIdx.z, cog = blockIdx.y;
    unsigned bid0 = blockIdx.x;
    if (P.xcd_remap) bid0 = (bid0 & 7) * (gridDim.x >> 3) + (bid0 >> 3);
    int bid = (int)bid0;
    const int tx = bid % P.tiles_x;
    bid /= P.tiles_x;
    const int ty = bid % P.tiles_y;
    const int b = bid / P.tiles_y;
    const int oy0 = ty * TH, ox0 = tx * NBW;
    const int S = P.nchunk * SPC;
    constexpr int R = pf_ring(MB, NPW, WM, WP, KH, KW, STR, TZ);
    static_assert(R >= 3, "no room for a weight ring");
    const unsigned lds0 = __builtin_amdgcn_readfirstlane((unsigned)(size_t)(const __attribute__((address_space(3))) uint4 *)smem_u);
    const unsigned wl_lds = lds0 + (unsigned)(NPB * PST) * 16u;

    const int Hp = P.H + 2, Wp = P.W + 2;
    const int iy0 = oy0 * STR - P.pad_y[z] + 1, ix0 = ox0 * STR - P.pad_x[z] + 1;
    unsigned xoff[KX];
#pragma unroll
    for (int i = 0; i < KX; ++i) {
        int e = (2 * i + (pwi & 1)) * 64 + lane;
        if (e >= NX) e = 0;
        const int q = e / PLANE, rem = e - q * PLANE;
        const int r = rem / PW, cp = rem - r * PW;
        const int c = STR == 2 ? (cp < NE ? 2 * cp : 2 * (cp - NE) + 1) : cp;
        const int iy = min(max(iy0 + r, 0), Hp - 1), ix = min(max(ix0 + c, 0), Wp - 1);
        xoff[i] = (unsigned)((q * Hp + iy) * Wp + ix) * 16u;
    }
    const long long cg_bytes = (long long)4 * Hp * Wp * 16;
    const char *s0 = reinterpret_cast<const char *>(P.src0) + (size_t)b * P.src0_bs * 16;
    const char *s1 = P.src1 ? reinterpret_cast<const char *>(P.src1) + (size_t)b * P.src1_bs * 16 : nullptr;
    const int c0_chunks = P.C0 >> 4;
    constexpr int ISSUE_TAPS = TAPS >= 9 ? 6 : (TAPS == 7 ? 5 : (TAPS >= 4 ? 2 : 1));
    constexpr int PER = (KX + ISSUE_TAPS - 1) / ISSUE_TAPS;
    auto issue_patch = [&](int chunk, auto tc) {
        constexpr int t = decltype(tc)::value;
        const char *base = chunk < c0_chunks ? s0 + (long long)chunk * cg_bytes : s1 + (long long)(chunk - c0_chunks) * cg_bytes;
        int pb = chunk;
        if constexpr (NPB == 2) pb &= 1; else pb %= 3;
        const unsigned dst = lds0 + (unsigned)(pb * PST) * 16u + (unsigned)(pwi & 1) * 1024u;
#pragma unroll
        for (int i = 0; i < KX; ++i)
            if (t < 0 || i / PER == t)
                if (2 * i + (pwi & 1) < XSW) dma16(xoff[i], base, dst + (unsigned)(2 * i) * 1024u);
    };
    const char *wsrc = reinterpret_cast<const char *>(P.w) + ((size_t)z * P.w_zs + (size_t)cog * COPT) * 16;
    unsigned wvo[NWW], wdo[NWW];
#pragma unroll
    for (int k = 0; k < NWW; ++k) {
        const int jj = min(wave + k * NWV, WI - 1);
        if constexpr (COPT == 32) {
            wvo[k] = (unsigned)(jj * 64 + lane) * 16u;
        } else {
            const int row = jj / (COPT / 64), seg = jj - row * (COPT / 64);
            wvo[k] = (unsigned)(row * P.COP + seg * 64 + lane) * 16u;
        }
        wdo[k] = __builtin_amdgcn_readfirstlane((unsigned)jj * 1024u);
    }
    const long long w_dt = (long long)P.nchunk * 6 * P.COP * 16;
    const long long w_dz = (long long)P.w_zs * 16 - (TAPZ - TPS) * w_dt;
    const long long w_dc = (long long)6 * P.COP * 16 - (TAPZ - TPS) * w_dt - (TZ - 1) * (long long)P.w_zs * 16;
    const char *wptr = wsrc;
    int tw = 0, sw = 0;
    auto issue_w = [&]() {
        const unsigned dst = wl_lds + (unsigned)(sw * WST) * 16u;
#pragma unroll
        for (int q = 0; q < TPS; ++q)
#pragma unroll
            for (int k = 0; k < NWW; ++k) dma16(wvo[k], wptr + q * w_dt, dst + (unsigned)(q * TAPW) * 16u + wdo[k]);
        tw += TPS;
        if (tw == TAPS) { tw = 0; wptr += w_dc; }
        else if (TZ > 1 && (tw % TAPZ) == 0) wptr += w_dz;
        else wptr += TPS * w_dt;
        if (++sw == R) sw = 0;
    };

    f32x16 acc[MB][NB], acc2[ACC2 ? MB : 1][ACC2 ? NB : 1];
#pragma unroll
    for (int m = 0; m < MB; ++m)
#pragma unroll
        for (int n = 0; n < NB; ++n)
#pragma unroll
            for (int r = 0; r < 16; ++r) {
                acc[m][n][r] = 0.f;
                if constexpr (ACC2) acc2[m][n][r] = 0.f;
            }

    const int half = lane >> 5, j = lane & 31;
    const int pr = 0, pc = j;
    const uint4 *a_base = smem_u + NPB * PST + half * COPT + wm * MB * 32 + j;
    const uint4 *b_base = smem_u + (half * 2) * PLANE + (wp * NPW * STR) * PW + j;

    typedef f16x8 OpsA[NPL][MB];
    typedef f16x8 OpsB[2][NPW];
    auto fetch = [&](auto tc, const uint4 *xb, const uint4 *wa, OpsA &A, OpsB &Bv) {
        constexpr int t = decltype(tc)::value;
        constexpr int tz = t % TAPZ, ph = t / TAPZ;
        constexpr int kx = tz % KW;
        constexpr int koff = TZ == 4 ? (tz / KW + (ph >> 1)) * PW + kx + (ph & 1)
                                     : (tz / KW) * PW + (STR == 2 ? (kx & 1) * NE + kx / 2 : kx);
#pragma unroll
        for (int pl = 0; pl < NPL; ++pl)
#pragma unroll
            for (int m = 0; m < MB; ++m) A[pl][m] = __builtin_bit_cast(f16x8, wa[(pl * 2) * COPT + m * 32]);
#pragma unroll
        for (int pl = 0; pl < 2; ++pl)
#pragma unroll
            for (int n = 0; n < NPW; ++n) Bv[pl][n] = __builtin_bit_cast(f16x8, xb[pl * PLANE + n * STR * PW + koff]);
    };
    auto mma = [&](const OpsA &A, const OpsB &Bv, auto phc) {
        constexpr int q0 = decltype(phc)::value * NPW;
        if constexpr (ACC2) {
#pragma unroll
            for (int m = 0; m < MB; ++m)
#pragma unroll
                for (int n = 0; n < NPW; ++n) acc[m][q0 + n] = __builtin_amdgcn_mfma_f32_32x32x16_f16(A[1][m], Bv[0][n], acc[m][q0 + n], 0, 0, 0);
#pragma unroll
            for (int m = 0; m < MB; ++m)
#pragma unroll
                for (int n = 0; n < NPW; ++n) acc2[m][q0 + n] = __builtin_amdgcn_mfma_f32_32x32x16_f16(A[0][m], Bv[1][n], acc2[m][q0 + n], 0, 0, 0);
#pragma unroll
            for (int m = 0; m < MB; ++m)
#pragma unroll
                for (int n = 0; n < NPW; ++n) acc[m][q0 + n] = __builtin_amdgcn_mfma_f32_32x32x16_f16(A[0][m], Bv[0][n], acc[m][q0 + n], 0, 0, 0);
        } else {
#pragma unroll
            for (int term = 0; term < 3; ++term) {
                constexpr int PA[3] = {1, 2, 0};
                constexpr int PB[3] = {0, 1, 0};
#pragma unroll
                for (int m = 0; m < MB; ++m)
#pragma unroll
                    for (int n = 0; n < NPW; ++n)
                        acc[m][q0 + n] = __builtin_amdgcn_mfma_f32_32x32x16_f16(A[PA[term] % NPL][m], Bv[PB[term]][n], acc[m][q0 + n], 0, 0, 0);
            }
        }
    };

    PFTL(0);
    if constexpr (UF != 0) {
        if (!patch_wave)
            for (int q = 0; q < R - 1 && q < S; ++q) issue_w();
        constexpr int XW = NBW + 6;
        float *xs = reinterpret_cast<float *>(smem_u + NPB * PST + R * WST);
        {
            constexpr int NS = (UF * PH * XW + NT - 1) / NT;
            float sv[NS];
#pragma unroll
            for (int k = 0; k < NS; ++k) {
                const int i = tid + k * NT;
                const int ci = i / (PH * XW), rem = i - ci * (PH * XW), r = rem / XW, cc = rem - r * XW;
                const int iy = oy0 - 3 + r, ix = ox0 - 3 + cc;
                sv[k] = (i < UF * PH * XW && iy >= 0 && iy < P.H && ix >= 0 && ix < P.W) ? P.x0[(size_t)b * P.x0_bs + ((size_t)ci * P.H + iy) * P.W + ix] : 0.f;
            }
#pragma unroll
            for (int k = 0; k < NS; ++k)
                if (tid + k * NT < UF * PH * XW) xs[tid + k * NT] = sv[k];
        }
        __syncthreads();
        for (int px = tid; px < PLANE; px += NT) {
            const int r = px / PW, c = px - r * PW;
            _Float16 hq[32], lq[32];
#pragma unroll
            for (int ch = 0; ch < 32; ++ch) {
                if (ch < 7 * UF) split2h(xs[((ch % UF) * PH + r) * XW + c + ch / UF], hq[ch], lq[ch]);
                else { hq[ch] = (_Float16)0.f; lq[ch] = (_Float16)0.f; }
            }
#pragma unroll
            for (int q = 0; q < 4; ++q) {
                f16x8 hv, lv;
#pragma unroll
                for (int t = 0; t < 8; ++t) { hv[t] = hq[8 * q + t]; lv[t] = lq[8 * q + t]; }
                uint4 *pbuf = smem_u + (q >> 1) * PST + ((q & 1) * 2) * PLANE + px;
                pbuf[0] = __builtin_bit_cast(uint4, hv);
                pbuf[PLANE] = __builtin_bit_cast(uint4, lv);
            }
        }
    } else if (patch_wave) {
        for (int c = 0; c < LA && c < P.nchunk; ++c) issue_patch(c, std::integral_constant<int, -1>{});
    } else {
        for (int q = 0; q < R - 1 && q < S; ++q) issue_w();
    }
    PFTL(1);
    dma_wait();
    __builtin_amdgcn_s_barrier();
    PFTL(2);
    OpsA A0, A1;
    OpsB B0, B1;
    fetch(std::integral_constant<int, 0>{}, b_base, a_base, A0, B0);
    int rem = S - 1;
    int sn = 0;
    auto tap = [&](auto tc, auto tailc, int chunk, const uint4 *xb_cur, const uint4 *xb_nxt, OpsA &Ac, OpsB &Bc, OpsA &An,
                   OpsB &Bn) {
        constexpr int t = decltype(tc)::value;
        constexpr bool TAIL = decltype(tailc)::value;
        constexpr bool SEND = (t % TPS) == TPS - 1;
        if constexpr (!SEND) {
            if (!(CDC_PF_ABLATE && (P.dbg & 64)))
                fetch(std::integral_constant<int, t + 1>{}, xb_cur, a_base + sn * WST + ((t + 1) % TPS) * TAPW, An, Bn);
            if (patch_wave) {
                if constexpr (t < ISSUE_TAPS)
                    if (UF == 0 && chunk + LA < P.nchunk && !(CDC_PF_ABLATE && (P.dbg & 2))) issue_patch(chunk + LA, tc);
            }
        } else {
        if (!(TAIL && t == TAPS - 1) || rem > 0) {
            if (++sn == R) sn = 0;
            if (CDC_PF_ABLATE && (P.dbg & 8)) {
            } else if (patch_wave) {
                if constexpr (t == TAPS - 1) {
                    if (LA == 2 && TAPS > 1 && chunk + LA < P.nchunk) vm_wait<XSW / 2>();
                    else dma_wait();
                }
            } else if (!TAIL || rem >= R - 2) {
                vm_wait<(R - 3 - (R >= 5 ? CDC_DMA_WAIT_MARGIN : 0)) * NWW * TPS>();
            } else {
                dma_wait();
            }
            if (!(CDC_PF_ABLATE && (P.dbg & 4))) __builtin_amdgcn_s_barrier();
            const uint4 *wa = a_base + sn * WST;
            if (CDC_PF_ABLATE && (P.dbg & 64)) {
            } else if constexpr (t == TAPS - 1) fetch(std::integral_constant<int, 0>{}, xb_nxt, wa, An, Bn);
            else fetch(std::integral_constant<int, t + 1>{}, xb_cur, wa, An, Bn);
            if (patch_wave) {
                if constexpr (t < ISSUE_TAPS)
                    if (UF == 0 && chunk + LA < P.nchunk && !(CDC_PF_ABLATE && (P.dbg & 2))) issue_patch(chunk + LA, tc);
            } else if ((!TAIL || rem >= R - 1) && !(CDC_PF_ABLATE && (P.dbg & 1))) {
                issue_w();
            }
        }
        --rem;
        }
        __builtin_amdgcn_s_setprio(2);
        if (!(CDC_PF_ABLATE && (P.dbg & 32))) mma(Ac, Bc, std::integral_constant<int, t / TAPZ>{});
        __builtin_amdgcn_s_setprio(0);
    };
    int pbc = 0;
    auto chunk_body = [&](auto parc, auto tailc, int chunk) {
        constexpr int par0 = decltype(parc)::value;
        int pbn = pbc + 1;
        if (pbn == NPB) pbn = 0;
        const uint4 *xb_cur = b_base + pbc * PST, *xb_nxt = b_base + pbn * PST;
        static_for<TAPS>([&](auto tc) {
            constexpr int t = decltype(tc)::value;
            if constexpr (((par0 + t) & 1) == 0) tap(tc, tailc, chunk, xb_cur, xb_nxt, A0, B0, A1, B1);
            else tap(tc, tailc, chunk, xb_cur, xb_nxt, A1, B1, A0, B0);
        });
        pbc = pbn;
    };
    using P0 = std::integral_constant<int, 0>;
    using P1 = std::integral_constant<int, 1>;
    const int n_main = max(0, min(P.nchunk - 1, (S - R + 1) / SPC));
    if constexpr ((TAPS & 1) == 0) {
        int chunk = 0;
        for (; chunk < n_main; ++chunk) chunk_body(P0{}, std::false_type{}, chunk);
        for (; chunk < P.nchunk; ++chunk) chunk_body(P0{}, std::true_type{}, chunk);
    } else {
        int chunk = 0;
        for (; chunk + 1 < n_main; chunk += 2) {
            chunk_body(P0{}, std::false_type{}, chunk);
            chunk_body(P1{}, std::false_type{}, chunk + 1);
        }
        for (; chunk + 1 < P.nchunk; chunk += 2) {
            chunk_body(P0{}, std::true_type{}, chunk);
            chunk_body(P1{}, std::true_type{}, chunk + 1);
        }
        if (chunk < P.nchunk) chunk_body(P0{}, std::true_type{}, chunk);
    }

    __builtin_amdgcn_s_barrier();
    PFTL(3);
    if (CDC_PF_ABLATE && (P.dbg & 256)) { PFTL_END(); return; }
    float *ep = reinterpret_cast<float *>(smem_u);
    float *red = ep + 4 * COPT;
    for (int i = tid; i < COPT; i += NT) {
        const int co = cog * COPT + i;
        const bool ok = co < P.Cout;
        ep[i] = (ok && P.bias) ? P.bias[co] : 0.f;
        ep[COPT + i] = (ok && P.ep_g) ? P.ep_g[co] : 0.f;
        ep[2 * COPT + i] = (ok && P.ep_b) ? P.ep_b[co] : 0.f;
        ep[3 * COPT + i] = (ok && P.shift) ? P.shift[(size_t)b * P.shift_bs + co] : 0.f;
    }
    __syncthreads();
    PFTL(4);
    const float inv_c = 1.0f / (float)P.Cout;
    const int cobase = cog * COPT + wm * MB * 32;
    const float *epl = ep + wm * MB * 32 + 4 * half;
    const bool ch_ok = cobase + MB * 32 <= P.Cout || COPT == 32;
    const int nvalid = P.Cout - cobase;
    if constexpr (TZ == 4) {
        if (!P.pre_add && !P.resid && !P.resid_pf && !P.res3_w && !P.relu && !P.shift && !P.stat_mean && (WM == 1 || !P.ep_g)) {
            static_assert(!ACC2, "fused phases: one accumulator set");
#pragma unroll
            for (int py = 0; py < 2; ++py)
#pragma unroll
                for (int n = 0; n < NPW; ++n) {
                    const int q0 = (py * 2) * NPW + n, q1 = q0 + NPW;
                    const int oy = oy0 + (wp * NPW + n) * NBH + pr, ox = ox0 + pc;
                    const bool valid = (oy < P.Ho) && (ox < P.Wo) && ch_ok;
                    int eo = 0;
                    asm volatile("" : "+v"(eo));
                    const float *eq = epl + eo;
#pragma unroll
                    for (int m = 0; m < MB; ++m)
#pragma unroll
                        for (int r = 0; r < 16; ++r) {
                            const float bi = eq[m * 32 + (r & 3) + 8 * (r >> 2)];
                            acc[m][q0][r] = acc[m][q0][r] * P.acc_scale + bi;
                            acc[m][q1][r] = acc[m][q1][r] * P.acc_scale + bi;
                        }
                    if constexpr (WM == 1) {
                        if (P.ep_g) {
                            float mean[2], rinv[2];
#pragma unroll
                            for (int i = 0; i < 2; ++i) {
                                const int q = i ? q1 : q0;
                                float sm = 0.f;
#pragma unroll
                                for (int m = 0; m < MB; ++m)
#pragma unroll
                                    for (int r = 0; r < 16; ++r) sm += acc[m][q][r];
                                sm += __shfl_xor(sm, 32);
                                mean[i] = sm * inv_c;
                                float sq = 0.f;
#pragma unroll
                                for (int m = 0; m < MB; ++m)
#pragma unroll
                                    for (int r = 0; r < 16; ++r) { const float d = acc[m][q][r] - mean[i]; sq += d * d; }
                                sq += __shfl_xor(sq, 32);
                                if (P.fault && !(sq < 3.0e38f)) *P.fault = 1;
                                rinv[i] = 1.0f / sqrtf(sq * inv_c + P.eps);
                            }
#pragma unroll
                            for (int m = 0; m < MB; ++m)
#pragma unroll
                                for (int r = 0; r < 16; ++r) {
                                    const int ci = m * 32 + (r & 3) + 8 * (r >> 2);
                                    const float gi = eq[COPT + ci], bi = eq[2 * COPT + ci];
                                    acc[m][q0][r] = (acc[m][q0][r] - mean[0]) * rinv[0] * gi + bi;
                                    acc[m][q1][r] = (acc[m][q1][r] - mean[1]) * rinv[1] * gi + bi;
                                }
                        }
                    }
                    if (!P.ep_g && P.fault) {
                        float sa = 0.f;
#pragma unroll
                        for (int m = 0; m < MB; ++m)
#pragma unroll
                            for (int r = 0; r < 16; ++r) sa += fabsf(acc[m][q0][r]) + fabsf(acc[m][q1][r]);
                        if (!(sa < 3.0e38f)) *P.fault = 1;
                    }
                    if (valid && !(CDC_PF_ABLATE && (P.dbg & 16))) {
                        if (P.out) {
                            float *op = P.out + (size_t)b * P.out_bs + (unsigned)(oy * P.out_ys + ox * P.out_xs + P.out_zoff[py * 2]) + (size_t)(cobase + 4 * half) * P.out_cs;
#pragma unroll
                            for (int m = 0; m < MB; ++m)
#pragma unroll
                                for (int r = 0; r < 16; ++r)
                                    *reinterpret_cast<float2 *>(op + (size_t)(m * 32 + (r & 3) + 8 * (r >> 2)) * P.out_cs) = make_float2(acc[m][q0][r], acc[m][q1][r]);
                        }
                        if (P.out_pf) {
                            const long long u0 = (long long)b * P.pf_bs + (long long)oy * P.pf_ys + (long long)ox * P.pf_xs + P.pf_zoff[py * 2] + half;
#pragma unroll
                            for (int m = 0; m < MB; ++m)
#pragma unroll
                                for (int g = 0; g < 4; ++g) {
                                    _Float16 h0[4], l0[4], h1[4], l1[4];
#pragma unroll
                                    for (int i = 0; i < 4; ++i) {
                                        split2h(acc[m][q0][g * 4 + i], h0[i], l0[i]);
                                        split2h(acc[m][q1][g * 4 + i], h1[i], l1[i]);
                                    }
                                    const f16x4 hv0 = {h0[0], h0[1], h0[2], h0[3]}, lv0 = {l0[0], l0[1], l0[2], l0[3]};
                                    const f16x4 hv1 = {h1[0], h1[1], h1[2], h1[3]}, lv1 = {l1[0], l1[1], l1[2], l1[3]};
                                    const uint2 a0 = __builtin_bit_cast(uint2, hv0), a1 = __builtin_bit_cast(uint2, hv1);
                                    const uint2 c0 = __builtin_bit_cast(uint2, lv0), c1 = __builtin_bit_cast(uint2, lv1);
                                    const uint2 sh = half ? a0 : a1, sl = half ? c0 : c1;
                                    uint2 rh, rl;
                                    rh.x = __shfl_xor(sh.x, 32); rh.y = __shfl_xor(sh.y, 32);
                                    rl.x = __shfl_xor(sl.x, 32); rl.y = __shfl_xor(sl.y, 32);
                                    const uint4 uh = half ? make_uint4(rh.x, rh.y, a1.x, a1.y) : make_uint4(a0.x, a0.y, rh.x, rh.y);
                                    const uint4 ul = half ? make_uint4(rl.x, rl.y, c1.x, c1.y) : make_uint4(c0.x, c0.y, rl.x, rl.y);
                                    uint4 *pu = reinterpret_cast<uint4 *>(P.out_pf) + u0 + (long long)((cobase >> 3) + m * 4 + g) * 2 * P.pf_ps;
                                    pu[0] = uh;
                                    pu[P.pf_ps] = ul;
                                }
                        }
                    }
                    __builtin_amdgcn_sched_barrier(0);
                }
            PFTL(6);
            PFTL_END();
            return;
        }
    }
    float mean_v[NB], rinv_v[NB];
    bool valid_v[NB];
    unsigned pix_v[NB];
#pragma unroll
    for (int n = 0; n < NB; ++n) {
        const int oy = oy0 + (wp * NPW + n % NPW) * NBH + pr, ox = ox0 + pc;
        const int zn = TZ == 4 ? n / NPW : z;
        valid_v[n] = (oy < P.Ho) && (ox < P.Wo) && ch_ok;
        pix_v[n] = (unsigned)(oy * P.out_ys + ox * P.out_xs + P.out_zoff[zn]);
        const float *eq = epl;
#pragma unroll
        for (int m = 0; m < MB; ++m)
#pragma unroll
            for (int r = 0; r < 16; ++r)
                acc[m][n][r] = (ACC2 ? acc[m][n][r] + acc2[ACC2 ? m : 0][ACC2 ? n : 0][r] * (1.0f / 2048.0f) : acc[m][n][r]) * P.acc_scale +
                               eq[m * 32 + (r & 3) + 8 * (r >> 2)];
        if (P.pre_add && P.pre_c4 && valid_v[n]) {
            const size_t hw = (size_t)P.Ho * P.Wo;
            const float4 *p4 = reinterpret_cast<const float4 *>(P.pre_add) + ((size_t)b * (P.Cout >> 2) + (cobase >> 2) + half) * hw + (size_t)oy * P.Wo + ox;
#pragma unroll
            for (int m = 0; m < MB; ++m)
#pragma unroll
                for (int g = 0; g < 4; ++g) {
                    const float4 v = p4[(size_t)(m * 8 + 2 * g) * hw];
                    acc[m][n][4 * g] += v.x; acc[m][n][4 * g + 1] += v.y; acc[m][n][4 * g + 2] += v.z; acc[m][n][4 * g + 3] += v.w;
                }
        } else if (P.pre_add && valid_v[n]) {
            const float *pp = P.pre_add + (size_t)b * P.out_bs + pix_v[n] + (size_t)(cobase + 4 * half) * P.out_cs;
#pragma unroll
            for (int m = 0; m < MB; ++m)
#pragma unroll
                for (int r = 0; r < 16; ++r) acc[m][n][r] += pp[(size_t)(m * 32 + (r & 3) + 8 * (r >> 2)) * P.out_cs];
        }
    }
    auto chan_stats = [&](float *mean_o, float *rinv_o) {
        const int slot = (wp * NB) * 32 + j;
        float part[NB];
#pragma unroll
        for (int n = 0; n < NB; ++n) {
            float sm = 0.f;
#pragma unroll
            for (int m = 0; m < MB; ++m)
#pragma unroll
                for (int r = 0; r < 16; ++r) sm += acc[m][n][r];
            sm += __shfl_xor(sm, 32);
            part[n] = sm;
        }
        if constexpr (WM > 1) {
            __syncthreads();
#pragma unroll
            for (int n = 0; n < NB; ++n)
                if (half == 0) red[wm * (WP * NB * 32) + slot + n * 32] = part[n];
            __syncthreads();
#pragma unroll
            for (int n = 0; n < NB; ++n) {
                float sm = 0.f;
#pragma unroll
                for (int q = 0; q < WM; ++q) sm += red[q * (WP * NB * 32) + slot + n * 32];
                part[n] = sm;
            }
        }
#pragma unroll
        for (int n = 0; n < NB; ++n) {
            mean_o[n] = part[n] * inv_c;
            float sq = 0.f;
#pragma unroll
            for (int m = 0; m < MB; ++m)
#pragma unroll
                for (int r = 0; r < 16; ++r) { const float d = acc[m][n][r] - mean_o[n]; sq += d * d; }
            sq += __shfl_xor(sq, 32);
            part[n] = sq;
        }
        if constexpr (WM > 1) {
            float *red2 = red + WM * (WP * NB * 32);
#pragma unroll
            for (int n = 0; n < NB; ++n)
                if (half == 0) red2[wm * (WP * NB * 32) + slot + n * 32] = part[n];
            __syncthreads();
#pragma unroll
            for (int n = 0; n < NB; ++n) {
                float sq = 0.f;
#pragma unroll
                for (int q = 0; q < WM; ++q) sq += red2[q * (WP * NB * 32) + slot + n * 32];
                part[n] = sq;
            }
        }
#pragma unroll
        for (int n = 0; n < NB; ++n) {
            if (P.fault && !(part[n] < 3.0e38f)) *P.fault = 1;
            rinv_o[n] = 1.0f / sqrtf(part[n] * inv_c + P.eps);
        }
    };
    if (P.ep_g) {
        chan_stats(mean_v, rinv_v);
#pragma unroll
        for (int n = 0; n < NB; ++n) {
            const float *eq = epl;
#pragma unroll
            for (int m = 0; m < MB; ++m)
#pragma unroll
                for (int r = 0; r < 16; ++r) {
                    const int ci = m * 32 + (r & 3) + 8 * (r >> 2);
                    acc[m][n][r] = (acc[m][n][r] - mean_v[n]) * rinv_v[n] * eq[COPT + ci] + eq[2 * COPT + ci];
                }
        }
    } else if (P.fault) {
#pragma unroll
        for (int n = 0; n < NB; ++n) {
            float s = 0.f;
#pragma unroll
            for (int m = 0; m < MB; ++m)
#pragma unroll
                for (int r = 0; r < 16; ++r) s += fabsf(acc[m][n][r]);
            if (!(s < 3.0e38f)) *P.fault = 1;
        }
    }
#pragma unroll
    for (int n = 0; n < NB; ++n) {
        if (P.relu) {
#pragma unroll
            for (int m = 0; m < MB; ++m)
#pragma unroll
                for (int r = 0; r < 16; ++r) acc[m][n][r] = fmaxf(acc[m][n][r], P.relu_slope * acc[m][n][r]);
        }
        if (P.shift) {
            const float *eq = epl;
#pragma unroll
            for (int m = 0; m < MB; ++m)
#pragma unroll
                for (int r = 0; r < 16; ++r) acc[m][n][r] += eq[3 * COPT + m * 32 + (r & 3) + 8 * (r >> 2)];
        }
        if (P.resid_pf && valid_v[n]) {
            const int oy = oy0 + (wp * NPW + n % NPW) * NBH + pr, ox = ox0 + pc;
            const uint2 *up = reinterpret_cast<const uint2 *>(reinterpret_cast<const uint4 *>(P.resid_pf) + (long long)b * P.rpf_bs + (long long)(cobase >> 3) * 2 * P.rpf_ps +
                                                              (long long)oy * P.rpf_ys + ox + P.rpf_zoff) + half;
#pragma unroll
            for (int m = 0; m < MB; ++m)
#pragma unroll
                for (int g = 0; g < 4; ++g) {
                    const uint2 hu = up[(long long)((m * 4 + g) * 2) * P.rpf_ps * 2], lu = up[(long long)((m * 4 + g) * 2 + 1) * P.rpf_ps * 2];
                    const f16x4 hv = __builtin_bit_cast(f16x4, hu), lv = __builtin_bit_cast(f16x4, lu);
#pragma unroll
                    for (int i = 0; i < 4; ++i) acc[m][n][g * 4 + i] += __builtin_fmaf((float)lv[i], 1.0f / 2048.0f, (float)hv[i]);
                }
        } else if (P.resid && valid_v[n]) {
            const float *rp = (P.resid1 && cobase >= P.resid_c0)
                                  ? P.resid1 + (size_t)b * P.resid1_bs + pix_v[n] + (size_t)(cobase - P.resid_c0 + 4 * half) * P.resid_cs
                                  : P.resid + (size_t)b * P.resid_bs + pix_v[n] + (size_t)(cobase + 4 * half) * P.resid_cs;
#pragma unroll
            for (int m = 0; m < MB; ++m)
#pragma unroll
                for (int r = 0; r < 16; ++r) acc[m][n][r] += rp[(size_t)(m * 32 + (r & 3) + 8 * (r >> 2)) * P.resid_cs];
        }
    }
    if (P.res3_w) {
        const size_t hw = (size_t)P.Ho * P.Wo;
#pragma unroll
        for (int n = 0; n < NB; ++n) {
            const int oy = oy0 + (wp * NPW + n % NPW) * NBH + pr, ox = ox0 + pc;
            const float *xp = P.res3_x + (size_t)b * P.res3_bs + (size_t)oy * P.Wo + ox;
            const float x0 = valid_v[n] ? xp[0] : 0.f, x1 = valid_v[n] ? xp[hw] : 0.f, x2 = valid_v[n] ? xp[2 * hw] : 0.f;
#pragma unroll
            for (int m = 0; m < MB; ++m)
#pragma unroll
                for (int r = 0; r < 16; ++r) {
                    const int co = cobase + m * 32 + (r & 3) + 8 * (r >> 2) + 4 * half;
                    acc[m][n][r] += P.res3_w[co] * x0 + P.res3_w[(size_t)P.COP + co] * x1 + P.res3_w[2 * (size_t)P.COP + co] * x2;
                }
        }
    }
    if (P.stat_mean) {
        chan_stats(mean_v, rinv_v);
#pragma unroll
        for (int n = 0; n < NB; ++n)
            if (valid_v[n] && half == 0 && wm == 0) {
                P.stat_mean[(size_t)b * P.out_cs + pix_v[n]] = mean_v[n];
                P.stat_rstd[(size_t)b * P.out_cs + pix_v[n]] = rinv_v[n];
            }
    }
    PFTL(5);
    if constexpr (TZ == 4) {
#pragma unroll
        for (int py = 0; py < 2; ++py)
#pragma unroll
            for (int n = 0; n < NPW; ++n) {
                const int q0 = (py * 2) * NPW + n, q1 = q0 + NPW;
                if (!valid_v[q0] || (CDC_PF_ABLATE && (P.dbg & 16))) continue;
                if (P.out) {
                    float *op = P.out + (size_t)b * P.out_bs + pix_v[q0] + (size_t)(cobase + 4 * half) * P.out_cs;
#pragma unroll
                    for (int m = 0; m < MB; ++m)
#pragma unroll
                        for (int r = 0; r < 16; ++r)
                            *reinterpret_cast<float2 *>(op + (size_t)(m * 32 + (r & 3) + 8 * (r >> 2)) * P.out_cs) = make_float2(acc[m][q0][r], acc[m][q1][r]);
                }
                if (P.out_pf) {
                    const int oy = oy0 + (wp * NPW + n) * NBH + pr, ox = ox0 + pc;
                    const long long u0 = (long long)b * P.pf_bs + (long long)oy * P.pf_ys + (long long)ox * P.pf_xs + P.pf_zoff[py * 2] + half;
#pragma unroll
                    for (int m = 0; m < MB; ++m)
#pragma unroll
                        for (int g = 0; g < 4; ++g) {
                            _Float16 h0[4], l0[4], h1[4], l1[4];
#pragma unroll
                            for (int i = 0; i < 4; ++i) {
                                split2h(acc[m][q0][g * 4 + i], h0[i], l0[i]);
                                split2h(acc[m][q1][g * 4 + i], h1[i], l1[i]);
                            }
                            const f16x4 hv0 = {h0[0], h0[1], h0[2], h0[3]}, lv0 = {l0[0], l0[1], l0[2], l0[3]};
                            const f16x4 hv1 = {h1[0], h1[1], h1[2], h1[3]}, lv1 = {l1[0], l1[1], l1[2], l1[3]};
                            const uint2 a0 = __builtin_bit_cast(uint2, hv0), a1 = __builtin_bit_cast(uint2, hv1);
                            const uint2 c0 = __builtin_bit_cast(uint2, lv0), c1 = __builtin_bit_cast(uint2, lv1);
                            const uint2 sh = half ? a0 : a1, sl = half ? c0 : c1;
                            uint2 rh, rl;
                            rh.x = __shfl_xor(sh.x, 32); rh.y = __shfl_xor(sh.y, 32);
                            rl.x = __shfl_xor(sl.x, 32); rl.y = __shfl_xor(sl.y, 32);
                            const uint4 uh = half ? make_uint4(rh.x, rh.y, a1.x, a1.y) : make_uint4(a0.x, a0.y, rh.x, rh.y);
                            const uint4 ul = half ? make_uint4(rl.x, rl.y, c1.x, c1.y) : make_uint4(c0.x, c0.y, rl.x, rl.y);
                            uint4 *pu = reinterpret_cast<uint4 *>(P.out_pf) + u0 + (long long)((cobase >> 3) + m * 4 + g) * 2 * P.pf_ps;
                            pu[0] = uh;
                            pu[P.pf_ps] = ul;
                        }
                }
            }
        PFTL(6);
        PFTL_END();
        return;
    }
#pragma unroll
    for (int n = 0; n < NB; ++n) {
        if (!valid_v[n] || (CDC_PF_ABLATE && (P.dbg & 16))) continue;
        if (P.out) {
            float *op = P.out + (size_t)b * P.out_bs + pix_v[n] + (size_t)(cobase + 4 * half) * P.out_cs;
#pragma unroll
            for (int m = 0; m < MB; ++m)
#pragma unroll
                for (int r = 0; r < 16; ++r) {
                    const int ci = m * 32 + (r & 3) + 8 * (r >> 2);
                    if (COPT != 32 || ci + 4 * half < nvalid) op[(size_t)ci * P.out_cs] = acc[m][n][r];
                }
        }
        if (P.out_pf) {
            const int oy = oy0 + (wp * NPW + n % NPW) * NBH + pr, ox = ox0 + pc;
            const long long u0 = (long long)b * P.pf_bs + (long long)oy * P.pf_ys + (long long)ox * P.pf_xs + P.pf_zoff[TZ == 4 ? n / NPW : z];
#pragma unroll
            for (int m = 0; m < MB; ++m)
                pf_store_block(reinterpret_cast<uint4 *>(P.out_pf), u0 + (long long)((cobase >> 3) + m * 4) * 2 * P.pf_ps, P.pf_ps, half, acc[m][n]);
        }
    }
    PFTL(6);
    PFTL_END();
}

typedef void (*pf_kernel_fn)(const PfArgs);

}
```

Measured before the change: 5.389.

## Add persistent-workgroup form to plane-format conv kernel for s2, TZ4 and 1x7 shapes

Adds a persistent mode to conv_pf_kernel. A grid sized to CU occupancy walks a contiguous range of tiles per workgroup and prefetches the next tile's patch and weights while the current tile's epilogue runs. The aim is to cut launch tail and the per-tile pipeline fill and drain for stride-2, TZ4 and 1x7 convs. In exchange it reserves extra LDS for epilogue staging, which shrinks the weight ring, and adds control complexity. The form is disabled for WM>1 with LN or stats epilogues.

New measurement: 4.306. -20.1%, worse.

```diff
diff --git a/cdc_compression_amd/csrc/cdc_internal.h b/cdc_compression_amd/csrc/cdc_internal.h
--- a/cdc_compression_amd/csrc/cdc_internal.h
+++ b/cdc_compression_amd/csrc/cdc_internal.h
@@ -55,6 +55,7 @@
     int MB, NPW, WM, WP, ring, tiles_x, tiles_y, groups; size_t lds_bytes; int lin = 0;
     int x16 = 0;
     int pf3_epv = 0, pf3_G = 0, pf3_iters = 0;
+    int pers = 0;
 };
 bool pf_make_plan(const PfShape &s, PfPlan *plan);
 hipError_t pf_launch(PfArgs a, const PfPlan &plan, int B, int nz, hipStream_t st);
diff --git a/cdc_compression_amd/csrc/cdc_planner.hip b/cdc_compression_amd/csrc/cdc_planner.hip
--- a/cdc_compression_amd/csrc/cdc_planner.hip
+++ b/cdc_compression_amd/csrc/cdc_planner.hip
@@ -27,10 +27,11 @@
                      op.conv.ep_g ? " LN" : "",
                      op.conv.ln_mean ? " pre" : "", cur == &h->pre_ops ? " HOIST" : "", op.conv.resid ? " +res" : "");
         else if (op.kind == Op::CONVPF)
-            snprintf(buf, sizeof buf, "conv %dx%d s%d %4d->%-4d out %3dx%-3d MB%d NPW%d WM%d WP%d g%d R%d %s%s%s%s%s%s", op.pf.KH, op.pf.KW,
+            snprintf(buf, sizeof buf, "conv %dx%d s%d %4d->%-4d out %3dx%-3d MB%d NPW%d WM%d WP%d g%d R%d %s%s%s%s%s%s%s", op.pf.KH, op.pf.KW,
                      op.pf.stride == 2 ? 2 : 1, op.pf.Cin, op.pf.Cout, op.pf.Ho, op.pf.Wo, op.pfplan.MB, op.pfplan.NPW, op.pfplan.WM, op.pfplan.WP,
                      op.pfplan.groups, op.pfplan.ring, op.pw ? (op.pf.pre_mean ? "PW pre" : "PW") : (op.pfplan.pf3_epv ? (op.pf.ep_g ? "PF3 LN" : "PF3") : (op.pf.ep_g ? "PF LN" : "PF")), op.pf.out ? "" : " nof32", op.pf.out_pf ? " +pf" : "",
-                     op.pf.resid ? " +res" : (op.pf.resid_pf ? " +resP" : ""), cur == &h->pre_ops ? " HOIST" : "", op.pf.tz == 4 ? " TZ4" : "");
+                     op.pf.resid ? " +res" : (op.pf.resid_pf ? " +resP" : ""), cur == &h->pre_ops ? " HOIST" : "", op.pf.tz == 4 ? " TZ4" : "",
+                     (!op.pw && !op.pfplan.pf3_epv && op.pfplan.pers) ? " pers" : "");
         else if (op.kind == Op::CONVWS)
             snprintf(buf, sizeof buf, "conv 3x3 s%d %4d->%-4d out %3dx%-3d NPB%d waves%d tiles%d g%d WS%s", op.wsplan.stride, op.ws.Cin, op.ws.Cout, op.ws.H, op.wsplan.W,
                      op.wsplan.NPB, op.wsplan.waves, op.wsplan.tiles, op.wsplan.groups, op.ws.pre_add ? " pre_add" : "");
@@ -348,6 +349,7 @@
                     a.resid_pf = tr->p; a.rpf_bs = tr->bs(); a.rpf_ps = tr->ps(); a.rpf_ys = Wo + 2; a.rpf_zoff = (Wo + 2) + 1;
                 }
             }
+        if (op.pfplan.WM > 1 && (a.ep_g || a.stat_mean)) op.pfplan.pers = 0;
         if (planB == 0) pf3_make_plan(a, B, w.nz, &op.pfplan);
         if (debug_plan())
             fprintf(stderr, "[plan] conv %dx%d %d->%d out %dx%d on conv_pf%s_kernel (epv %d, %d workgroups x %d tiles per group)\n", w.KH, w.KW, w.Cin, w.Cout,
diff --git a/cdc_compression_amd/csrc/conv_inst_p.hip b/cdc_compression_amd/csrc/conv_inst_p.hip
--- a/cdc_compression_amd/csrc/conv_inst_p.hip
+++ b/cdc_compression_amd/csrc/conv_inst_p.hip
@@ -19,25 +19,29 @@
     if (MB == 2 && NPW == 2 && WM == 4 && WP == 2) return conv_pf_kernel<2, 2, 4, 2, KH, KW>;
     return nullptr;
 }
+template <bool PERS>
 static pf_kernel_fn pf_lookup_s2(int MB, int NPW, int WM, int WP) {
-    if (MB == 2 && NPW == 1 && WM == 1 && WP == 4) return conv_pf_kernel<2, 1, 1, 4, 3, 3, 2>;
-    if (MB == 2 && NPW == 2 && WM == 2 && WP == 2) return conv_pf_kernel<2, 2, 2, 2, 3, 3, 2>;
-    if (MB == 3 && NPW == 1 && WM == 2 && WP == 4) return conv_pf_kernel<3, 1, 2, 4, 3, 3, 2>;
+    if (MB == 2 && NPW == 1 && WM == 1 && WP == 4) return conv_pf_kernel<2, 1, 1, 4, 3, 3, 2, 1, 0, PERS>;
+    if (MB == 2 && NPW == 2 && WM == 2 && WP == 2) return conv_pf_kernel<2, 2, 2, 2, 3, 3, 2, 1, 0, PERS>;
+    if (MB == 3 && NPW == 1 && WM == 2 && WP == 4) return conv_pf_kernel<3, 1, 2, 4, 3, 3, 2, 1, 0, PERS>;
     return nullptr;
 }
+template <bool PERS>
 static pf_kernel_fn pf_lookup_tz(int MB, int NPW, int WM, int WP) {
-    if (MB == 1 && NPW == 2 && WM == 2 && WP == 2) return conv_pf_kernel<1, 2, 2, 2, 2, 2, 1, 4>;
-    if (MB == 2 && NPW == 1 && WM == 1 && WP == 4) return conv_pf_kernel<2, 1, 1, 4, 2, 2, 1, 4>;
-    if (MB == 1 && NPW == 2 && WM == 4 && WP == 2) return conv_pf_kernel<1, 2, 4, 2, 2, 2, 1, 4>;
+    if (MB == 1 && NPW == 2 && WM == 2 && WP == 2) return conv_pf_kernel<1, 2, 2, 2, 2, 2, 1, 4, 0, PERS>;
+    if (MB == 2 && NPW == 1 && WM == 1 && WP == 4) return conv_pf_kernel<2, 1, 1, 4, 2, 2, 1, 4, 0, PERS>;
+    if (MB == 1 && NPW == 2 && WM == 4 && WP == 2) return conv_pf_kernel<1, 2, 4, 2, 2, 2, 1, 4, 0, PERS>;
     return nullptr;
 }
-static pf_kernel_fn pf_lookup(int MB, int NPW, int WM, int WP, int KH, int KW, int stride = 1, int tz = 1) {
-    if (tz == 4) return (KH == 2 && KW == 2 && stride != 2) ? pf_lookup_tz(MB, NPW, WM, WP) : nullptr;
-    if (stride == 2) return (KH == 3 && KW == 3) ? pf_lookup_s2(MB, NPW, WM, WP) : nullptr;
+static pf_kernel_fn pf_lookup(int MB, int NPW, int WM, int WP, int KH, int KW, int stride = 1, int tz = 1, bool pers = false) {
+    if (tz == 4) return (KH == 2 && KW == 2 && stride != 2) ? (pers ? pf_lookup_tz<true>(MB, NPW, WM, WP) : pf_lookup_tz<false>(MB, NPW, WM, WP)) : nullptr;
+    if (stride == 2) return (KH == 3 && KW == 3) ? (pers ? pf_lookup_s2<true>(MB, NPW, WM, WP) : pf_lookup_s2<false>(MB, NPW, WM, WP)) : nullptr;
+    if (KH == 1 && KW == 7 && MB == 1 && NPW == 2 && WM == 1 && WP == 4)
+        return pers ? conv_pf_kernel<1, 2, 1, 4, 1, 7, 1, 1, 0, true> : conv_pf_kernel<1, 2, 1, 4, 1, 7>;
+    if (pers) return nullptr;
     if (KH == 3 && KW == 3) return pf_lookup_k<3, 3>(MB, NPW, WM, WP);
     if (KH == 1 && KW == 1) return pf_lookup_k<1, 1>(MB, NPW, WM, WP);
     if (KH == 2 && KW == 2) return pf_lookup_k<2, 2>(MB, NPW, WM, WP);
-    if (KH == 1 && KW == 7 && MB == 1 && NPW == 2 && WM == 1 && WP == 4) return conv_pf_kernel<1, 2, 1, 4, 1, 7>;
     if (KH == 7 && KW == 1 && MB == 2 && NPW == 2 && WM == 1 && WP == 4) return conv_pf_kernel<2, 2, 1, 4, 7, 1, 1, 1, 3>;
     return nullptr;
 }
@@ -62,7 +66,22 @@
     {2, 2, 1, 4},
 };
 
+constexpr long long kPfPersMinTiles = 2;
+constexpr int kPfPersForms = 7;
+static int pf_pers_wgs(const PfPlan &p, int B, int bound_per_cu, int form) {
+    if (dev_env("CDC_NO_PF_PERS")) return 0;
+    const int forms = dev_env("CDC_PF_PERS_FORMS") ? atoi(dev_env("CDC_PF_PERS_FORMS")) : kPfPersForms;
+    if (!(forms & form)) return 0;
+    if (const char *e = dev_env("CDC_PF_PERS_WGS")) return std::max(0, atoi(e));
+    const long long tiles = (long long)p.tiles_x * p.tiles_y * B;
+    const int per_cu = std::max(1, std::min(bound_per_cu, (int)((160 * 1024) / p.lds_bytes)));
+    long long G = (long long)device_cus() * per_cu / std::max(1, p.groups);
+    if (G >= 64) G &= ~7ll;
+    return (G >= 1 && tiles >= kPfPersMinTiles * G) ? (int)G : 0;
+}
+
 bool pf_make_plan(const PfShape &s, PfPlan *p) {
+    p->pers = 0;
     if (s.uf) {
         if (s.uf != 3 || s.KH != 7 || s.KW != 1 || s.Cin != 21 || s.Cout != 64 || s.cop != 64 || s.C0 || s.nz != 1 || s.stride != 1 || s.tz != 1 ||
             s.Wo < 32 || dev_env("CDC_NO_PF_UF"))
@@ -86,7 +105,8 @@
         if (!ring || (s.Cin / 16) * 7 < ring - 1 || wgs < min_wgs) return false;
         p->MB = 1; p->NPW = 2; p->WM = 1; p->WP = 4; p->ring = ring;
         p->tiles_x = (s.Wo + 31) / 32; p->tiles_y = (s.Ho + 7) / 8; p->groups = 1;
-        p->lds_bytes = (size_t)2 * pf_patch_units(2, 4, 1, 7) * 16 + (size_t)ring * pf_rows(1, 2) * 32 * 16;
+        p->lds_bytes = (size_t)2 * pf_patch_units(2, 4, 1, 7) * 16 + (size_t)ring * pf_rows(1, 2) * 32 * 16 + pf_pers_ep_bytes(1, 1);
+        p->pers = pf_pers_wgs(*p, s.B, 3, 4);
         return true;
     }
     if (s.Cout % 32 || s.Cin % 16 || (s.C0 % 16)) return false;
@@ -116,8 +136,9 @@
             p->ring = ring;
             p->tiles_x = (s.Wo + 31) / 32; p->tiles_y = (s.Ho + TH - 1) / TH;
             p->groups = s.Cout / COPT;
-            p->lds_bytes = std::max(patch + ring * wst, sizeof(float) * (size_t)(4 * COPT + 2 * c.WM * c.WP * c.NPW * 32));
+            p->lds_bytes = std::max(patch + ring * wst + pf_pers_ep_bytes(c.MB, c.WM), sizeof(float) * (size_t)(4 * COPT + 2 * c.WM * c.WP * c.NPW * 32));
         }
+        if (best >= 0) p->pers = pf_pers_wgs(*p, s.B, 1, 1);
         return best >= 0;
     }
     if (s.tz == 4) {
@@ -139,7 +160,8 @@
             p->ring = ring;
             p->tiles_x = (s.Wo + 31) / 32; p->tiles_y = (s.Ho + TH - 1) / TH;
             p->groups = 1;
-            p->lds_bytes = std::max(patch + ring * wst, sizeof(float) * (size_t)(4 * COPT + 2 * c.WM * c.WP * 4 * c.NPW * 32));
+            p->lds_bytes = std::max(patch + ring * wst + pf_pers_ep_bytes(c.MB, c.WM), sizeof(float) * (size_t)(4 * COPT + 2 * c.WM * c.WP * 4 * c.NPW * 32));
+            p->pers = pf_pers_wgs(*p, s.B, 2, 2);
             break;
         }
         return best >= 0;
@@ -180,14 +202,16 @@
 
 hipError_t pf_launch(PfArgs a, const PfPlan &p, int B, int nz, hipStream_t st) {
     if (p.pf3_epv) return pf3_launch(a, p, B, st);
-    pf_kernel_fn fn = pf_lookup(p.MB, p.NPW, p.WM, p.WP, a.KH, a.KW, a.stride == 2 ? 2 : 1, a.tz == 4 ? 4 : 1);
+    const bool pers = p.pers > 0;
+    if (pers && p.WM > 1 && (a.ep_g || a.stat_mean)) return hipErrorInvalidValue;
+    pf_kernel_fn fn = pf_lookup(p.MB, p.NPW, p.WM, p.WP, a.KH, a.KW, a.stride == 2 ? 2 : 1, a.tz == 4 ? 4 : 1, pers);
     if (!fn) return hipErrorInvalidValue;
     if (a.tz == 4) nz = 1;
     a.lognbw = 5;
     a.dbg = 0;
     a.tiles_x = p.tiles_x; a.tiles_y = p.tiles_y; a.B = B; a.ring = p.ring;
     if (hipError_t e = ensure_dynamic_lds((const void *)fn, p.lds_bytes); e != hipSuccess) return e;
-    dim3 grid((unsigned)(p.tiles_x * p.tiles_y * B), (unsigned)p.groups, (unsigned)nz);
+    dim3 grid((unsigned)(pers ? p.pers : p.tiles_x * p.tiles_y * B), (unsigned)p.groups, (unsigned)nz);
     a.xcd_remap = (grid.x % 8 == 0 && grid.x >= 64) ? 1 : 0;
 #ifdef CDC_TIMELINE
     static unsigned long long *tl_dev = nullptr;
diff --git a/cdc_compression_amd/csrc/conv_pf_kernel.h b/cdc_compression_amd/csrc/conv_pf_kernel.h
--- a/cdc_compression_amd/csrc/conv_pf_kernel.h
+++ b/cdc_compression_amd/csrc/conv_pf_kernel.h
@@ -8,6 +8,9 @@
 
 #ifndef CDC_DMA_WAIT_MARGIN
 #define CDC_DMA_WAIT_MARGIN 1
+#endif
+#ifndef CDC_PF_R4_MARGIN
+#define CDC_PF_R4_MARGIN 0
 #endif
 #ifdef CDC_DMA_WAIT_ALL
 constexpr int kVmWaitMask = 0;
@@ -38,8 +41,11 @@
 #define CDC_PF_S2_NPB 2
 #endif
 __host__ __device__ constexpr int pf_patch_bufs(int KH, int KW, int STR = 1) { return STR == 2 ? CDC_PF_S2_NPB : (KH * KW == 1 ? 3 : 2); }
+__host__ __device__ constexpr bool pf_has_pers(int KH, int KW, int STR, int TZ) { return STR == 2 || TZ == 4 || (KH == 1 && KW == 7); }
+__host__ __device__ constexpr int pf_pers_ep_bytes(int MB, int WM) { return 4 * WM * MB * 32 * 4; }
 __host__ __device__ constexpr int pf_ring_tps(int MB, int NPW, int WM, int WP, int KH, int KW, int STR, int tps, int TZ = 1) {
-    const size_t budget = ((WM * WP == 8 || STR == 2) ? 156 * 1024 : 80 * 1024) - ((KH == 7 && KW == 1) ? pf_uf_stage_floats(NPW, WP) * 4 : 0);
+    const size_t budget = ((WM * WP == 8 || STR == 2) ? 156 * 1024 : 80 * 1024) - ((KH == 7 && KW == 1) ? pf_uf_stage_floats(NPW, WP) * 4 : 0) -
+                          (pf_has_pers(KH, KW, STR, TZ) ? pf_pers_ep_bytes(MB, WM) : 0);
     const size_t patch = (size_t)pf_patch_bufs(KH, KW, STR) * pf_patch_units(NPW, WP, KH, KW, STR, TZ) * 16;
     const size_t wst = (size_t)tps * pf_rows(MB, TZ * NPW) * WM * MB * 32 * 16;
 #ifndef CDC_PF_RING_MAX
@@ -69,7 +75,7 @@
 #define CDC_PF_ABLATE 0
 #endif
 
-template <int MB, int NPW, int WM, int WP, int KH, int KW, int STR = 1, int TZ = 1, int UF = 0>
+template <int MB, int NPW, int WM, int WP, int KH, int KW, int STR = 1, int TZ = 1, int UF = 0, bool PERS = false>
 __global__ void __launch_bounds__(64 * WM * WP, (KH == 1 && KW == 7) ? 3 : STR == 2 ? 1 : ((WM * WP == 8 || MB * NPW * TZ <= 4 || (TZ == 4 && MB * NPW <= 2 && CDC_PF_TZ_MINB == 2)) ? 2 : 1)) conv_pf_kernel(const PfArgs P) {
     constexpr int NW = WM * WP, NT = 64 * NW, COPT = WM * MB * 32;
     static_assert(COPT % 64 == 0 || COPT == 32, "a weight DMA instruction (64 units) must stay inside one (plane, k-half) row");
@@ -111,20 +117,45 @@
 #define PFTL(c) do { } while (0)
 #define PFTL_END() do { } while (0)
 #endif
-    const int tid = threadIdx.x, lane = tid & 63;
+    const int tid = threadIdx.x;
+    int lane = tid & 63;
     const int wave = __builtin_amdgcn_readfirstlane(tid >> 6);
     const int wm = wave / WP, wp = wave % WP;
     const bool patch_wave = wave >= NWV;
     const int pwi = wave - NWV;
     const int z = blockIdx.z, cog = blockIdx.y;
+    static_assert(!PERS || (UF == 0 && pf_has_pers(KH, KW, STR, TZ) && pf_patch_bufs(KH, KW, STR) == 2), "persistent form: plane-tensor patches, two patch buffers");
     unsigned bid0 = blockIdx.x;
     if (P.xcd_remap) bid0 = (bid0 & 7) * (gridDim.x >> 3) + (bid0 >> 3);
-    int bid = (int)bid0;
-    const int tx = bid % P.tiles_x;
-    bid /= P.tiles_x;
-    const int ty = bid % P.tiles_y;
-    const int b = bid / P.tiles_y;
-    const int oy0 = ty * TH, ox0 = tx * NBW;
+    int b, oy0, ox0;
+    int tiles_left = 1;
+    if constexpr (PERS) {
+        const long long T = (long long)P.tiles_x * P.tiles_y * P.B;
+        const int t_lo = (int)(bid0 * T / gridDim.x), t_hi = (int)((bid0 + 1) * T / gridDim.x);
+        tiles_left = t_hi - t_lo;
+        if (tiles_left <= 0) return;
+        const int txy = P.tiles_x * P.tiles_y;
+        b = t_lo / txy;
+        const int r = t_lo - b * txy, tx = r / P.tiles_y;
+        oy0 = (r - tx * P.tiles_y) * TH;
+        ox0 = tx * NBW;
+    } else {
+        int bid = (int)bid0;
+        const int tx = bid % P.tiles_x;
+        bid /= P.tiles_x;
+        const int ty = bid % P.tiles_y;
+        b = bid / P.tiles_y;
+        oy0 = ty * TH;
+        ox0 = tx * NBW;
+    }
+    auto next_tile = [&](int &b_, int &oy_, int &ox_) {
+        oy_ += TH;
+        if (oy_ >= P.tiles_y * TH) {
+            oy_ = 0;
+            ox_ += NBW;
+            if (ox_ >= P.tiles_x * NBW) { ox_ = 0; ++b_; }
+        }
+    };
     const int S = P.nchunk * SPC;
     constexpr int R = pf_ring(MB, NPW, WM, WP, KH, KW, STR, TZ);
     static_assert(R >= 3, "no room for a weight ring");
@@ -132,53 +163,69 @@
     const unsigned wl_lds = lds0 + (unsigned)(NPB * PST) * 16u;
 
     const int Hp = P.H + 2, Wp = P.W + 2;
-    const int iy0 = oy0 * STR - P.pad_y[z] + 1, ix0 = ox0 * STR - P.pad_x[z] + 1;
+    constexpr bool XREC = PERS && TZ == 4;
     unsigned xoff[KX];
-#pragma unroll
-    for (int i = 0; i < KX; ++i) {
+    const char *s0, *s1;
+    int piy0 = 0, pix0 = 0;
+    auto patch_off = [&](int i, int iy0, int ix0) {
         int e = (2 * i + (pwi & 1)) * 64 + lane;
         if (e >= NX) e = 0;
         const int q = e / PLANE, rem = e - q * PLANE;
         const int r = rem / PW, cp = rem - r * PW;
         const int c = STR == 2 ? (cp < NE ? 2 * cp : 2 * (cp - NE) + 1) : cp;
         const int iy = min(max(iy0 + r, 0), Hp - 1), ix = min(max(ix0 + c, 0), Wp - 1);
-        xoff[i] = (unsigned)((q * Hp + iy) * Wp + ix) * 16u;
-    }
+        return (unsigned)((q * Hp + iy) * Wp + ix) * 16u;
+    };
+    auto set_patch_src = [&](int b_, int oy_, int ox_) {
+        const int iy0 = oy_ * STR - P.pad_y[z] + 1, ix0 = ox_ * STR - P.pad_x[z] + 1;
+        if constexpr (XREC) { piy0 = iy0; pix0 = ix0; }
+        else {
+#pragma unroll
+            for (int i = 0; i < KX; ++i) xoff[i] = patch_off(i, iy0, ix0);
+        }
+        s0 = reinterpret_cast<const char *>(P.src0) + (size_t)b_ * P.src0_bs * 16;
+        s1 = P.src1 ? reinterpret_cast<const char *>(P.src1) + (size_t)b_ * P.src1_bs * 16 : nullptr;
+    };
+    set_patch_src(b, oy0, ox0);
     const long long cg_bytes = (long long)4 * Hp * Wp * 16;
-    const char *s0 = reinterpret_cast<const char *>(P.src0) + (size_t)b * P.src0_bs * 16;
-    const char *s1 = P.src1 ? reinterpret_cast<const char *>(P.src1) + (size_t)b * P.src1_bs * 16 : nullptr;
     const int c0_chunks = P.C0 >> 4;
+    int pbc = 0;
     constexpr int ISSUE_TAPS = TAPS >= 9 ? 6 : (TAPS == 7 ? 5 : (TAPS >= 4 ? 2 : 1));
     constexpr int PER = (KX + ISSUE_TAPS - 1) / ISSUE_TAPS;
     auto issue_patch = [&](int chunk, auto tc) {
         constexpr int t = decltype(tc)::value;
         const char *base = chunk < c0_chunks ? s0 + (long long)chunk * cg_bytes : s1 + (long long)(chunk - c0_chunks) * cg_bytes;
         int pb = chunk;
-        if constexpr (NPB == 2) pb &= 1; else pb %= 3;
+        if constexpr (PERS) pb = t < 0 ? chunk : pbc ^ 1;
+        else if constexpr (NPB == 2) pb &= 1; else pb %= 3;
         const unsigned dst = lds0 + (unsigned)(pb * PST) * 16u + (unsigned)(pwi & 1) * 1024u;
 #pragma unroll
         for (int i = 0; i < KX; ++i)
             if (t < 0 || i / PER == t)
-                if (2 * i + (pwi & 1) < XSW) dma16(xoff[i], base, dst + (unsigned)(2 * i) * 1024u);
+                if (2 * i + (pwi & 1) < XSW) dma16(XREC ? patch_off(i, piy0, pix0) : xoff[i], base, dst + (unsigned)(2 * i) * 1024u);
     };
     const char *wsrc = reinterpret_cast<const char *>(P.w) + ((size_t)z * P.w_zs + (size_t)cog * COPT) * 16;
     unsigned wvo[NWW], wdo[NWW];
-#pragma unroll
-    for (int k = 0; k < NWW; ++k) {
-        const int jj = min(wave + k * NWV, WI - 1);
-        if constexpr (COPT == 32) {
-            wvo[k] = (unsigned)(jj * 64 + lane) * 16u;
-        } else {
-            const int row = jj / (COPT / 64), seg = jj - row * (COPT / 64);
-            wvo[k] = (unsigned)(row * P.COP + seg * 64 + lane) * 16u;
-        }
-        wdo[k] = __builtin_amdgcn_readfirstlane((unsigned)jj * 1024u);
-    }
+    auto set_w_off = [&]() {
+#pragma unroll
+        for (int k = 0; k < NWW; ++k) {
+            const int jj = min(wave + k * NWV, WI - 1);
+            if constexpr (COPT == 32) {
+                wvo[k] = (unsigned)(jj * 64 + lane) * 16u;
+            } else {
+                const int row = jj / (COPT / 64), seg = jj - row * (COPT / 64);
+                wvo[k] = (unsigned)(row * P.COP + seg * 64 + lane) * 16u;
+            }
+            wdo[k] = __builtin_amdgcn_readfirstlane((unsigned)jj * 1024u);
+        }
+    };
+    set_w_off();
     const long long w_dt = (long long)P.nchunk * 6 * P.COP * 16;
     const long long w_dz = (long long)P.w_zs * 16 - (TAPZ - TPS) * w_dt;
     const long long w_dc = (long long)6 * P.COP * 16 - (TAPZ - TPS) * w_dt - (TZ - 1) * (long long)P.w_zs * 16;
     const char *wptr = wsrc;
     int tw = 0, sw = 0;
+    int cw = 0;
     auto issue_w = [&]() {
         const unsigned dst = wl_lds + (unsigned)(sw * WST) * 16u;
 #pragma unroll
@@ -186,7 +233,12 @@
 #pragma unroll
             for (int k = 0; k < NWW; ++k) dma16(wvo[k], wptr + q * w_dt, dst + (unsigned)(q * TAPW) * 16u + wdo[k]);
         tw += TPS;
-        if (tw == TAPS) { tw = 0; wptr += w_dc; }
+        if (tw == TAPS) {
+            tw = 0;
+            wptr += w_dc;
+            if constexpr (PERS)
+                if (++cw == P.nchunk) { cw = 0; wptr = wsrc; }
+        }
         else if (TZ > 1 && (tw % TAPZ) == 0) wptr += w_dz;
         else wptr += TPS * w_dt;
         if (++sw == R) sw = 0;
@@ -203,8 +255,7 @@
                 if constexpr (ACC2) acc2[m][n][r] = 0.f;
             }
 
-    const int half = lane >> 5, j = lane & 31;
-    const int pr = 0, pc = j;
+    int half = lane >> 5, j = lane & 31;
     const uint4 *a_base = smem_u + NPB * PST + half * COPT + wm * MB * 32 + j;
     const uint4 *b_base = smem_u + (half * 2) * PLANE + (wp * NPW * STR) * PW + j;
 
@@ -298,15 +349,43 @@
     } else {
         for (int q = 0; q < R - 1 && q < S; ++q) issue_w();
     }
+    int b_shift = b;
+    auto load_ep = [&](float *ep, bool all) {
+        for (int i = tid; i < COPT; i += NT) {
+            const int co = cog * COPT + i;
+            const bool ok = co < P.Cout;
+            if (all) {
+                ep[i] = (ok && P.bias) ? P.bias[co] : 0.f;
+                ep[COPT + i] = (ok && P.ep_g) ? P.ep_g[co] : 0.f;
+                ep[2 * COPT + i] = (ok && P.ep_b) ? P.ep_b[co] : 0.f;
+            }
+            ep[3 * COPT + i] = (ok && P.shift) ? P.shift[(size_t)b * P.shift_bs + co] : 0.f;
+        }
+    };
+    if constexpr (PERS) load_ep(reinterpret_cast<float *>(smem_u + NPB * PST + R * WST), true);
     PFTL(1);
     dma_wait();
-    __builtin_amdgcn_s_barrier();
+    if constexpr (PERS) __syncthreads();
+    else __builtin_amdgcn_s_barrier();
     PFTL(2);
     OpsA A0, A1;
     OpsB B0, B1;
     fetch(std::integral_constant<int, 0>{}, b_base, a_base, A0, B0);
-    int rem = S - 1;
+    int rem = tiles_left * S - 1;
+    bool more = false;
+    bool last_chunk = false;
+    int skipw = 0;
     int sn = 0;
+    auto patch_ahead = [&](int chunk, auto tc) {
+        int nx = chunk + LA;
+        if constexpr (PERS) {
+            if (nx >= P.nchunk) {
+                if (!more) return;
+                nx -= P.nchunk;
+            }
+        } else if (nx >= P.nchunk) return;
+        if (UF == 0 && !(CDC_PF_ABLATE && (P.dbg & 2))) issue_patch(nx, tc);
+    };
     auto tap = [&](auto tc, auto tailc, int chunk, const uint4 *xb_cur, const uint4 *xb_nxt, OpsA &Ac, OpsB &Bc, OpsA &An,
                    OpsB &Bn) {
         constexpr int t = decltype(tc)::value;
@@ -317,7 +396,7 @@
                 fetch(std::integral_constant<int, t + 1>{}, xb_cur, a_base + sn * WST + ((t + 1) % TPS) * TAPW, An, Bn);
             if (patch_wave) {
                 if constexpr (t < ISSUE_TAPS)
-                    if (UF == 0 && chunk + LA < P.nchunk && !(CDC_PF_ABLATE && (P.dbg & 2))) issue_patch(chunk + LA, tc);
+                    patch_ahead(chunk, tc);
             }
         } else {
         if (!(TAIL && t == TAPS - 1) || rem > 0) {
@@ -328,19 +407,23 @@
                     if (LA == 2 && TAPS > 1 && chunk + LA < P.nchunk) vm_wait<XSW / 2>();
                     else dma_wait();
                 }
+            } else if (PERS && skipw > 0) {
+                --skipw;
             } else if (!TAIL || rem >= R - 2) {
-                vm_wait<(R - 3 - (R >= 5 ? CDC_DMA_WAIT_MARGIN : 0)) * NWW * TPS>();
+                vm_wait<(R - 3 - ((R >= 5 || CDC_PF_R4_MARGIN) ? CDC_DMA_WAIT_MARGIN : 0)) * NWW * TPS>();
             } else {
                 dma_wait();
             }
             if (!(CDC_PF_ABLATE && (P.dbg & 4))) __builtin_amdgcn_s_barrier();
             const uint4 *wa = a_base + sn * WST;
             if (CDC_PF_ABLATE && (P.dbg & 64)) {
-            } else if constexpr (t == TAPS - 1) fetch(std::integral_constant<int, 0>{}, xb_nxt, wa, An, Bn);
+            } else if constexpr (t == TAPS - 1) {
+                if (!(PERS && last_chunk)) fetch(std::integral_constant<int, 0>{}, xb_nxt, wa, An, Bn);
+            }
             else fetch(std::integral_constant<int, t + 1>{}, xb_cur, wa, An, Bn);
             if (patch_wave) {
                 if constexpr (t < ISSUE_TAPS)
-                    if (UF == 0 && chunk + LA < P.nchunk && !(CDC_PF_ABLATE && (P.dbg & 2))) issue_patch(chunk + LA, tc);
+                    patch_ahead(chunk, tc);
             } else if ((!TAIL || rem >= R - 1) && !(CDC_PF_ABLATE && (P.dbg & 1))) {
                 issue_w();
             }
@@ -351,7 +434,6 @@
         if (!(CDC_PF_ABLATE && (P.dbg & 32))) mma(Ac, Bc, std::integral_constant<int, t / TAPZ>{});
         __builtin_amdgcn_s_setprio(0);
     };
-    int pbc = 0;
     auto chunk_body = [&](auto parc, auto tailc, int chunk) {
         constexpr int par0 = decltype(parc)::value;
         int pbn = pbc + 1;
@@ -366,8 +448,28 @@
     };
     using P0 = std::integral_constant<int, 0>;
     using P1 = std::integral_constant<int, 1>;
-    const int n_main = max(0, min(P.nchunk - 1, (S - R + 1) / SPC));
-    if constexpr ((TAPS & 1) == 0) {
+    const int n_main = PERS ? max(0, min(tiles_left * P.nchunk - 1, (tiles_left * S - R + 1) / SPC)) : max(0, min(P.nchunk - 1, (S - R + 1) / SPC));
+    int par = 0, gch = 0;
+    int bn = b, oyn = oy0, oxn = ox0;
+    for (;;) {
+    if constexpr (PERS) {
+        more = tiles_left > 1;
+        for (int chunk = 0; chunk < P.nchunk; ++chunk, ++gch) {
+            last_chunk = chunk == P.nchunk - 1;
+            if (last_chunk && more) {
+                next_tile(bn, oyn, oxn);
+                if (patch_wave) set_patch_src(bn, oyn, oxn);
+            }
+            if (gch < n_main) {
+                if ((TAPS & 1) == 0 || par == 0) chunk_body(P0{}, std::false_type{}, chunk);
+                else chunk_body(P1{}, std::false_type{}, chunk);
+            } else {
+                if ((TAPS & 1) == 0 || par == 0) chunk_body(P0{}, std::true_type{}, chunk);
+                else chunk_body(P1{}, std::true_type{}, chunk);
+            }
+            par ^= (TAPS & 1);
+        }
+    } else if constexpr ((TAPS & 1) == 0) {
         int chunk = 0;
         for (; chunk < n_main; ++chunk) chunk_body(P0{}, std::false_type{}, chunk);
         for (; chunk < P.nchunk; ++chunk) chunk_body(P0{}, std::true_type{}, chunk);
@@ -384,28 +486,43 @@
         if (chunk < P.nchunk) chunk_body(P0{}, std::true_type{}, chunk);
     }
 
-    __builtin_amdgcn_s_barrier();
+    do {
+    const auto *pe = [&] {
+        if constexpr (PERS) {
+            const __attribute__((address_space(4))) PfArgs *q = (const __attribute__((address_space(4))) PfArgs *)__builtin_amdgcn_kernarg_segment_ptr();
+            asm volatile("" : "+s"(q));
+            return q;
+        } else return &P;
+    }();
+    if constexpr (!PERS) __builtin_amdgcn_s_barrier();
     PFTL(3);
-    if (CDC_PF_ABLATE && (P.dbg & 256)) { PFTL_END(); return; }
-    float *ep = reinterpret_cast<float *>(smem_u);
+    if (CDC_PF_ABLATE && (pe->dbg & 256)) { if constexpr (PERS) break; else { PFTL_END(); return; } }
+    float *ep = reinterpret_cast<float *>(PERS ? smem_u + NPB * PST + R * WST : smem_u);
     float *red = ep + 4 * COPT;
-    for (int i = tid; i < COPT; i += NT) {
-        const int co = cog * COPT + i;
-        const bool ok = co < P.Cout;
-        ep[i] = (ok && P.bias) ? P.bias[co] : 0.f;
-        ep[COPT + i] = (ok && P.ep_g) ? P.ep_g[co] : 0.f;
-        ep[2 * COPT + i] = (ok && P.ep_b) ? P.ep_b[co] : 0.f;
-        ep[3 * COPT + i] = (ok && P.shift) ? P.shift[(size_t)b * P.shift_bs + co] : 0.f;
-    }
-    __syncthreads();
+    const int pr = 0, pc = j;
+    if constexpr (!PERS) {
+        for (int i = tid; i < COPT; i += NT) {
+            const int co = cog * COPT + i;
+            const bool ok = co < pe->Cout;
+            ep[i] = (ok && pe->bias) ? pe->bias[co] : 0.f;
+            ep[COPT + i] = (ok && pe->ep_g) ? pe->ep_g[co] : 0.f;
+            ep[2 * COPT + i] = (ok && pe->ep_b) ? pe->ep_b[co] : 0.f;
+            ep[3 * COPT + i] = (ok && pe->shift) ? pe->shift[(size_t)b * pe->shift_bs + co] : 0.f;
+        }
+        __syncthreads();
+    } else if (pe->shift && b != b_shift) {
+        load_ep(ep, false);
+        b_shift = b;
+        __syncthreads();
+    }
     PFTL(4);
-    const float inv_c = 1.0f / (float)P.Cout;
+    const float inv_c = 1.0f / (float)pe->Cout;
     const int cobase = cog * COPT + wm * MB * 32;
     const float *epl = ep + wm * MB * 32 + 4 * half;
-    const bool ch_ok = cobase + MB * 32 <= P.Cout || COPT == 32;
-    const int nvalid = P.Cout - cobase;
+    const bool ch_ok = cobase + MB * 32 <= pe->Cout || COPT == 32;
+    const int nvalid = pe->Cout - cobase;
     if constexpr (TZ == 4) {
-        if (!P.pre_add && !P.resid && !P.resid_pf && !P.res3_w && !P.relu && !P.shift && !P.stat_mean && (WM == 1 || !P.ep_g)) {
+        if (!pe->pre_add && !pe->resid && !pe->resid_pf && !pe->res3_w && !pe->relu && !pe->shift && !pe->stat_mean && (WM == 1 || !pe->ep_g)) {
             static_assert(!ACC2, "fused phases: one accumulator set");
 #pragma unroll
             for (int py = 0; py < 2; ++py)
@@ -413,7 +530,7 @@
                 for (int n = 0; n < NPW; ++n) {
                     const int q0 = (py * 2) * NPW + n, q1 = q0 + NPW;
                     const int oy = oy0 + (wp * NPW + n) * NBH + pr, ox = ox0 + pc;
-                    const bool valid = (oy < P.Ho) && (ox < P.Wo) && ch_ok;
+                    const bool valid = (oy < pe->Ho) && (ox < pe->Wo) && ch_ok;
                     int eo = 0;
                     asm volatile("" : "+v"(eo));
                     const float *eq = epl + eo;
@@ -422,11 +539,11 @@
 #pragma unroll
                         for (int r = 0; r < 16; ++r) {
                             const float bi = eq[m * 32 + (r & 3) + 8 * (r >> 2)];
-                            acc[m][q0][r] = acc[m][q0][r] * P.acc_scale + bi;
-                            acc[m][q1][r] = acc[m][q1][r] * P.acc_scale + bi;
+                            acc[m][q0][r] = acc[m][q0][r] * pe->acc_scale + bi;
+                            acc[m][q1][r] = acc[m][q1][r] * pe->acc_scale + bi;
                         }
                     if constexpr (WM == 1) {
-                        if (P.ep_g) {
+                        if (pe->ep_g) {
                             float mean[2], rinv[2];
 #pragma unroll
                             for (int i = 0; i < 2; ++i) {
@@ -444,8 +561,8 @@
 #pragma unroll
                                     for (int r = 0; r < 16; ++r) { const float d = acc[m][q][r] - mean[i]; sq += d * d; }
                                 sq += __shfl_xor(sq, 32);
-                                if (P.fault && !(sq < 3.0e38f)) *P.fault = 1;
-                                rinv[i] = 1.0f / sqrtf(sq * inv_c + P.eps);
+                                if (pe->fault && !(sq < 3.0e38f)) *pe->fault = 1;
+                                rinv[i] = 1.0f / sqrtf(sq * inv_c + pe->eps);
                             }
 #pragma unroll
                             for (int m = 0; m < MB; ++m)
@@ -458,25 +575,26 @@
                                 }
                         }
                     }
-                    if (!P.ep_g && P.fault) {
+                    if (!pe->ep_g && pe->fault) {
                         float sa = 0.f;
 #pragma unroll
                         for (int m = 0; m < MB; ++m)
 #pragma unroll
                             for (int r = 0; r < 16; ++r) sa += fabsf(acc[m][q0][r]) + fabsf(acc[m][q1][r]);
-                        if (!(sa < 3.0e38f)) *P.fault = 1;
+                        if (!(sa < 3.0e38f)) *pe->fault = 1;
                     }
-                    if (valid && !(CDC_PF_ABLATE && (P.dbg & 16))) {
-                        if (P.out) {
-                            float *op = P.out + (size_t)b * P.out_bs + (unsigned)(oy * P.out_ys + ox * P.out_xs + P.out_zoff[py * 2]) + (size_t)(cobase + 4 * half) * P.out_cs;
+                    if (PERS && py == 0 && n == 0) dma_wait();
+                    if (valid && !(CDC_PF_ABLATE && (pe->dbg & 16))) {
+                        if (pe->out) {
+                            float *op = pe->out + (size_t)b * pe->out_bs + (unsigned)(oy * pe->out_ys + ox * pe->out_xs + pe->out_zoff[py * 2]) + (size_t)(cobase + 4 * half) * pe->out_cs;
 #pragma unroll
                             for (int m = 0; m < MB; ++m)
 #pragma unroll
                                 for (int r = 0; r < 16; ++r)
-                                    *reinterpret_cast<float2 *>(op + (size_t)(m * 32 + (r & 3) + 8 * (r >> 2)) * P.out_cs) = make_float2(acc[m][q0][r], acc[m][q1][r]);
+                                    *reinterpret_cast<float2 *>(op + (size_t)(m * 32 + (r & 3) + 8 * (r >> 2)) * pe->out_cs) = make_float2(acc[m][q0][r], acc[m][q1][r]);
                         }
-                        if (P.out_pf) {
-                            const long long u0 = (long long)b * P.pf_bs + (long long)oy * P.pf_ys + (long long)ox * P.pf_xs + P.pf_zoff[py * 2] + half;
+                        if (pe->out_pf) {
+                            const long long u0 = (long long)b * pe->pf_bs + (long long)oy * pe->pf_ys + (long long)ox * pe->pf_xs + pe->pf_zoff[py * 2] + half;
 #pragma unroll
                             for (int m = 0; m < MB; ++m)
 #pragma unroll
@@ -497,17 +615,16 @@
                                     rl.x = __shfl_xor(sl.x, 32); rl.y = __shfl_xor(sl.y, 32);
                                     const uint4 uh = half ? make_uint4(rh.x, rh.y, a1.x, a1.y) : make_uint4(a0.x, a0.y, rh.x, rh.y);
                                     const uint4 ul = half ? make_uint4(rl.x, rl.y, c1.x, c1.y) : make_uint4(c0.x, c0.y, rl.x, rl.y);
-                                    uint4 *pu = reinterpret_cast<uint4 *>(P.out_pf) + u0 + (long long)((cobase >> 3) + m * 4 + g) * 2 * P.pf_ps;
+                                    uint4 *pu = reinterpret_cast<uint4 *>(pe->out_pf) + u0 + (long long)((cobase >> 3) + m * 4 + g) * 2 * pe->pf_ps;
                                     pu[0] = uh;
-                                    pu[P.pf_ps] = ul;
+                                    pu[pe->pf_ps] = ul;
                                 }
                         }
                     }
                     __builtin_amdgcn_sched_barrier(0);
                 }
             PFTL(6);
-            PFTL_END();
-            return;
+            if constexpr (PERS) break; else { PFTL_END(); return; }
         }
     }
     float mean_v[NB], rinv_v[NB];
@@ -517,18 +634,18 @@
     for (int n = 0; n < NB; ++n) {
         const int oy = oy0 + (wp * NPW + n % NPW) * NBH + pr, ox = ox0 + pc;
         const int zn = TZ == 4 ? n / NPW : z;
-        valid_v[n] = (oy < P.Ho) && (ox < P.Wo) && ch_ok;
-        pix_v[n] = (unsigned)(oy * P.out_ys + ox * P.out_xs + P.out_zoff[zn]);
+        valid_v[n] = (oy < pe->Ho) && (ox < pe->Wo) && ch_ok;
+        pix_v[n] = (unsigned)(oy * pe->out_ys + ox * pe->out_xs + pe->out_zoff[zn]);
         const float *eq = epl;
 #pragma unroll
         for (int m = 0; m < MB; ++m)
 #pragma unroll
             for (int r = 0; r < 16; ++r)
-                acc[m][n][r] = (ACC2 ? acc[m][n][r] + acc2[ACC2 ? m : 0][ACC2 ? n : 0][r] * (1.0f / 2048.0f) : acc[m][n][r]) * P.acc_scale +
+                acc[m][n][r] = (ACC2 ? acc[m][n][r] + acc2[ACC2 ? m : 0][ACC2 ? n : 0][r] * (1.0f / 2048.0f) : acc[m][n][r]) * pe->acc_scale +
                                eq[m * 32 + (r & 3) + 8 * (r >> 2)];
-        if (P.pre_add && P.pre_c4 && valid_v[n]) {
-            const size_t hw = (size_t)P.Ho * P.Wo;
-            const float4 *p4 = reinterpret_cast<const float4 *>(P.pre_add) + ((size_t)b * (P.Cout >> 2) + (cobase >> 2) + half) * hw + (size_t)oy * P.Wo + ox;
+        if (pe->pre_add && pe->pre_c4 && valid_v[n]) {
+            const size_t hw = (size_t)pe->Ho * pe->Wo;
+            const float4 *p4 = reinterpret_cast<const float4 *>(pe->pre_add) + ((size_t)b * (pe->Cout >> 2) + (cobase >> 2) + half) * hw + (size_t)oy * pe->Wo + ox;
 #pragma unroll
             for (int m = 0; m < MB; ++m)
 #pragma unroll
@@ -536,12 +653,12 @@
                     const float4 v = p4[(size_t)(m * 8 + 2 * g) * hw];
                     acc[m][n][4 * g] += v.x; acc[m][n][4 * g + 1] += v.y; acc[m][n][4 * g + 2] += v.z; acc[m][n][4 * g + 3] += v.w;
                 }
-        } else if (P.pre_add && valid_v[n]) {
-            const float *pp = P.pre_add + (size_t)b * P.out_bs + pix_v[n] + (size_t)(cobase + 4 * half) * P.out_cs;
-#pragma unroll
-            for (int m = 0; m < MB; ++m)
-#pragma unroll
-                for (int r = 0; r < 16; ++r) acc[m][n][r] += pp[(size_t)(m * 32 + (r & 3) + 8 * (r >> 2)) * P.out_cs];
+        } else if (pe->pre_add && valid_v[n]) {
+            const float *pp = pe->pre_add + (size_t)b * pe->out_bs + pix_v[n] + (size_t)(cobase + 4 * half) * pe->out_cs;
+#pragma unroll
+            for (int m = 0; m < MB; ++m)
+#pragma unroll
+                for (int r = 0; r < 16; ++r) acc[m][n][r] += pp[(size_t)(m * 32 + (r & 3) + 8 * (r >> 2)) * pe->out_cs];
         }
     }
     auto chan_stats = [&](float *mean_o, float *rinv_o) {
@@ -598,11 +715,11 @@
         }
 #pragma unroll
         for (int n = 0; n < NB; ++n) {
-            if (P.fault && !(part[n] < 3.0e38f)) *P.fault = 1;
-            rinv_o[n] = 1.0f / sqrtf(part[n] * inv_c + P.eps);
-        }
-    };
-    if (P.ep_g) {
+            if (pe->fault && !(part[n] < 3.0e38f)) *pe->fault = 1;
+            rinv_o[n] = 1.0f / sqrtf(part[n] * inv_c + pe->eps);
+        }
+    };
+    if (pe->ep_g) {
         chan_stats(mean_v, rinv_v);
 #pragma unroll
         for (int n = 0; n < NB; ++n) {
@@ -615,7 +732,7 @@
                     acc[m][n][r] = (acc[m][n][r] - mean_v[n]) * rinv_v[n] * eq[COPT + ci] + eq[2 * COPT + ci];
                 }
         }
-    } else if (P.fault) {
+    } else if (pe->fault) {
 #pragma unroll
         for (int n = 0; n < NB; ++n) {
             float s = 0.f;
@@ -623,91 +740,92 @@
             for (int m = 0; m < MB; ++m)
 #pragma unroll
                 for (int r = 0; r < 16; ++r) s += fabsf(acc[m][n][r]);
-            if (!(s < 3.0e38f)) *P.fault = 1;
+            if (!(s < 3.0e38f)) *pe->fault = 1;
         }
     }
 #pragma unroll
     for (int n = 0; n < NB; ++n) {
-        if (P.relu) {
-#pragma unroll
-            for (int m = 0; m < MB; ++m)
-#pragma unroll
-                for (int r = 0; r < 16; ++r) acc[m][n][r] = fmaxf(acc[m][n][r], P.relu_slope * acc[m][n][r]);
-        }
-        if (P.shift) {
+        if (pe->relu) {
+#pragma unroll
+            for (int m = 0; m < MB; ++m)
+#pragma unroll
+                for (int r = 0; r < 16; ++r) acc[m][n][r] = fmaxf(acc[m][n][r], pe->relu_slope * acc[m][n][r]);
+        }
+        if (pe->shift) {
             const float *eq = epl;
 #pragma unroll
             for (int m = 0; m < MB; ++m)
 #pragma unroll
                 for (int r = 0; r < 16; ++r) acc[m][n][r] += eq[3 * COPT + m * 32 + (r & 3) + 8 * (r >> 2)];
         }
-        if (P.resid_pf && valid_v[n]) {
+        if (pe->resid_pf && valid_v[n]) {
             const int oy = oy0 + (wp * NPW + n % NPW) * NBH + pr, ox = ox0 + pc;
-            const uint2 *up = reinterpret_cast<const uint2 *>(reinterpret_cast<const uint4 *>(P.resid_pf) + (long long)b * P.rpf_bs + (long long)(cobase >> 3) * 2 * P.rpf_ps +
-                                                              (long long)oy * P.rpf_ys + ox + P.rpf_zoff) + half;
+            const uint2 *up = reinterpret_cast<const uint2 *>(reinterpret_cast<const uint4 *>(pe->resid_pf) + (long long)b * pe->rpf_bs + (long long)(cobase >> 3) * 2 * pe->rpf_ps +
+                                                              (long long)oy * pe->rpf_ys + ox + pe->rpf_zoff) + half;
 #pragma unroll
             for (int m = 0; m < MB; ++m)
 #pragma unroll
                 for (int g = 0; g < 4; ++g) {
-                    const uint2 hu = up[(long long)((m * 4 + g) * 2) * P.rpf_ps * 2], lu = up[(long long)((m * 4 + g) * 2 + 1) * P.rpf_ps * 2];
+                    const uint2 hu = up[(long long)((m * 4 + g) * 2) * pe->rpf_ps * 2], lu = up[(long long)((m * 4 + g) * 2 + 1) * pe->rpf_ps * 2];
                     const f16x4 hv = __builtin_bit_cast(f16x4, hu), lv = __builtin_bit_cast(f16x4, lu);
 #pragma unroll
                     for (int i = 0; i < 4; ++i) acc[m][n][g * 4 + i] += __builtin_fmaf((float)lv[i], 1.0f / 2048.0f, (float)hv[i]);
                 }
-        } else if (P.resid && valid_v[n]) {
-            const float *rp = (P.resid1 && cobase >= P.resid_c0)
-                                  ? P.resid1 + (size_t)b * P.resid1_bs + pix_v[n] + (size_t)(cobase - P.resid_c0 + 4 * half) * P.resid_cs
-                                  : P.resid + (size_t)b * P.resid_bs + pix_v[n] + (size_t)(cobase + 4 * half) * P.resid_cs;
-#pragma unroll
-            for (int m = 0; m < MB; ++m)
-#pragma unroll
-                for (int r = 0; r < 16; ++r) acc[m][n][r] += rp[(size_t)(m * 32 + (r & 3) + 8 * (r >> 2)) * P.resid_cs];
-        }
-    }
-    if (P.res3_w) {
-        const size_t hw = (size_t)P.Ho * P.Wo;
+        } else if (pe->resid && valid_v[n]) {
+            const float *rp = (pe->resid1 && cobase >= pe->resid_c0)
+                                  ? pe->resid1 + (size_t)b * pe->resid1_bs + pix_v[n] + (size_t)(cobase - pe->resid_c0 + 4 * half) * pe->resid_cs
+                                  : pe->resid + (size_t)b * pe->resid_bs + pix_v[n] + (size_t)(cobase + 4 * half) * pe->resid_cs;
+#pragma unroll
+            for (int m = 0; m < MB; ++m)
+#pragma unroll
+                for (int r = 0; r < 16; ++r) acc[m][n][r] += rp[(size_t)(m * 32 + (r & 3) + 8 * (r >> 2)) * pe->resid_cs];
+        }
+    }
+    if (pe->res3_w) {
+        const size_t hw = (size_t)pe->Ho * pe->Wo;
 #pragma unroll
         for (int n = 0; n < NB; ++n) {
             const int oy = oy0 + (wp * NPW + n % NPW) * NBH + pr, ox = ox0 + pc;
-            const float *xp = P.res3_x + (size_t)b * P.res3_bs + (size_t)oy * P.Wo + ox;
+            const float *xp = pe->res3_x + (size_t)b * pe->res3_bs + (size_t)oy * pe->Wo + ox;
             const float x0 = valid_v[n] ? xp[0] : 0.f, x1 = valid_v[n] ? xp[hw] : 0.f, x2 = valid_v[n] ? xp[2 * hw] : 0.f;
 #pragma unroll
             for (int m = 0; m < MB; ++m)
 #pragma unroll
                 for (int r = 0; r < 16; ++r) {
                     const int co = cobase + m * 32 + (r & 3) + 8 * (r >> 2) + 4 * half;
-                    acc[m][n][r] += P.res3_w[co] * x0 + P.res3_w[(size_t)P.COP + co] * x1 + P.res3_w[2 * (size_t)P.COP + co] * x2;
+                    acc[m][n][r] += pe->res3_w[co] * x0 + pe->res3_w[(size_t)pe->COP + co] * x1 + pe->res3_w[2 * (size_t)pe->COP + co] * x2;
                 }
         }
     }
-    if (P.stat_mean) {
+    if (pe->stat_mean) {
         chan_stats(mean_v, rinv_v);
 #pragma unroll
         for (int n = 0; n < NB; ++n)
             if (valid_v[n] && half == 0 && wm == 0) {
-                P.stat_mean[(size_t)b * P.out_cs + pix_v[n]] = mean_v[n];
-                P.stat_rstd[(size_t)b * P.out_cs + pix_v[n]] = rinv_v[n];
+                pe->stat_mean[(size_t)b * pe->out_cs + pix_v[n]] = mean_v[n];
+                pe->stat_rstd[(size_t)b * pe->out_cs + pix_v[n]] = rinv_v[n];
             }
     }
     PFTL(5);
+    if constexpr (PERS) dma_wait();
     if constexpr (TZ == 4) {
 #pragma unroll
         for (int py = 0; py < 2; ++py)
 #pragma unroll
             for (int n = 0; n < NPW; ++n) {
                 const int q0 = (py * 2) * NPW + n, q1 = q0 + NPW;
-                if (!valid_v[q0] || (CDC_PF_ABLATE && (P.dbg & 16))) continue;
-                if (P.out) {
-                    float *op = P.out + (size_t)b * P.out_bs + pix_v[q0] + (size_t)(cobase + 4 * half) * P.out_cs;
+                if (!valid_v[q0] || (CDC_PF_ABLATE && (pe->dbg & 16))) continue;
+                if (pe->out) {
+                    float *op = pe->out + (size_t)b * pe->out_bs + pix_v[q0] + (size_t)(cobase + 4 * half) * pe->out_cs;
 #pragma unroll
                     for (int m = 0; m < MB; ++m)
 #pragma unroll
                         for (int r = 0; r < 16; ++r)
-                            *reinterpret_cast<float2 *>(op + (size_t)(m * 32 + (r & 3) + 8 * (r >> 2)) * P.out_cs) = make_float2(acc[m][q0][r], acc[m][q1][r]);
+                            *reinterpret_cast<float2 *>(op + (size_t)(m * 32 + (r & 3) + 8 * (r >> 2)) * pe->out_cs) = make_float2(acc[m][q0][r], acc[m][q1][r]);
                 }
-                if (P.out_pf) {
+                if (pe->out_pf) {
                     const int oy = oy0 + (wp * NPW + n) * NBH + pr, ox = ox0 + pc;
-                    const long long u0 = (long long)b * P.pf_bs + (long long)oy * P.pf_ys + (long long)ox * P.pf_xs + P.pf_zoff[py * 2] + half;
+                    const long long u0 = (long long)b * pe->pf_bs + (long long)oy * pe->pf_ys + (long long)ox * pe->pf_xs + pe->pf_zoff[py * 2] + half;
 #pragma unroll
                     for (int m = 0; m < MB; ++m)
 #pragma unroll
@@ -728,38 +846,63 @@
                             rl.x = __shfl_xor(sl.x, 32); rl.y = __shfl_xor(sl.y, 32);
                             const uint4 uh = half ? make_uint4(rh.x, rh.y, a1.x, a1.y) : make_uint4(a0.x, a0.y, rh.x, rh.y);
                             const uint4 ul = half ? make_uint4(rl.x, rl.y, c1.x, c1.y) : make_uint4(c0.x, c0.y, rl.x, rl.y);
-                            uint4 *pu = reinterpret_cast<uint4 *>(P.out_pf) + u0 + (long long)((cobase >> 3) + m * 4 + g) * 2 * P.pf_ps;
+                            uint4 *pu = reinterpret_cast<uint4 *>(pe->out_pf) + u0 + (long long)((cobase >> 3) + m * 4 + g) * 2 * pe->pf_ps;
                             pu[0] = uh;
-                            pu[P.pf_ps] = ul;
+                            pu[pe->pf_ps] = ul;
                         }
                 }
             }
         PFTL(6);
-        PFTL_END();
-        return;
+        if constexpr (PERS) break; else { PFTL_END(); return; }
     }
 #pragma unroll
     for (int n = 0; n < NB; ++n) {
-        if (!valid_v[n] || (CDC_PF_ABLATE && (P.dbg & 16))) continue;
-        if (P.out) {
-            float *op = P.out + (size_t)b * P.out_bs + pix_v[n] + (size_t)(cobase + 4 * half) * P.out_cs;
+        if (!valid_v[n] || (CDC_PF_ABLATE && (pe->dbg & 16))) continue;
+        if (pe->out) {
+            float *op = pe->out + (size_t)b * pe->out_bs + pix_v[n] + (size_t)(cobase + 4 * half) * pe->out_cs;
 #pragma unroll
             for (int m = 0; m < MB; ++m)
 #pragma unroll
                 for (int r = 0; r < 16; ++r) {
                     const int ci = m * 32 + (r & 3) + 8 * (r >> 2);
-                    if (COPT != 32 || ci + 4 * half < nvalid) op[(size_t)ci * P.out_cs] = acc[m][n][r];
+                    if (COPT != 32 || ci + 4 * half < nvalid) op[(size_t)ci * pe->out_cs] = acc[m][n][r];
                 }
         }
-        if (P.out_pf) {
+        if (pe->out_pf) {
             const int oy = oy0 + (wp * NPW + n % NPW) * NBH + pr, ox = ox0 + pc;
-            const long long u0 = (long long)b * P.pf_bs + (long long)oy * P.pf_ys + (long long)ox * P.pf_xs + P.pf_zoff[TZ == 4 ? n / NPW : z];
-#pragma unroll
-            for (int m = 0; m < MB; ++m)
-                pf_store_block(reinterpret_cast<uint4 *>(P.out_pf), u0 + (long long)((cobase >> 3) + m * 4) * 2 * P.pf_ps, P.pf_ps, half, acc[m][n]);
+            const long long u0 = (long long)b * pe->pf_bs + (long long)oy * pe->pf_ys + (long long)ox * pe->pf_xs + pe->pf_zoff[TZ == 4 ? n / NPW : z];
+#pragma unroll
+            for (int m = 0; m < MB; ++m)
+                pf_store_block(reinterpret_cast<uint4 *>(pe->out_pf), u0 + (long long)((cobase >> 3) + m * 4) * 2 * pe->pf_ps, pe->pf_ps, half, acc[m][n]);
         }
     }
     PFTL(6);
+    } while (0);
+    if constexpr (!PERS) break;
+    else {
+        if (!more) break;
+        --tiles_left;
+        b = bn; oy0 = oyn; ox0 = oxn;
+        skipw = R - 2;
+        asm volatile("" : "+v"(lane));
+        half = lane >> 5; j = lane & 31;
+        a_base = smem_u + NPB * PST + half * COPT + wm * MB * 32 + j;
+        b_base = smem_u + (half * 2) * PLANE + (wp * NPW * STR) * PW + j;
+        set_w_off();
+        set_patch_src(b, oy0, ox0);
+#pragma unroll
+        for (int m = 0; m < MB; ++m)
+#pragma unroll
+            for (int n = 0; n < NB; ++n)
+#pragma unroll
+                for (int r = 0; r < 16; ++r) {
+                    acc[m][n][r] = 0.f;
+                    if constexpr (ACC2) acc2[m][n][r] = 0.f;
+                }
+        if ((TAPS & 1) == 0 || par == 0) fetch(std::integral_constant<int, 0>{}, b_base + pbc * PST, a_base + sn * WST, A0, B0);
+        else fetch(std::integral_constant<int, 0>{}, b_base + pbc * PST, a_base + sn * WST, A1, B1);
+    }
+    }
     PFTL_END();
 }
 
```
